# xandergos/terrain-diffusion

Hardware: AMD Instinct MI355X
Metric: terrain megapixels/sec (decoded) at fixed steps, 30m model (higher is better)
Workload: dtype bf16; 1 GPU; BASELINE configs[2]: terrain-diffusion-30m base U-Net, 8x8 tile grid (stride 32, 288x288 latents) with overlap blending, 20 steps, 64 windows batched per solver step; edm_steps=20, parallelism=1 independent streams (one process per GPU, no data-path collective)

## Files before the change

include/td_engine.h:

```cpp
#ifndef TD_ENGINE_H
#define TD_ENGINE_H
#include <stdint.h>

#ifdef __cplusplus
extern "C" {
#endif

typedef struct td_engine td_engine;
typedef struct td_unet td_unet;

enum { TD_OK = 0, TD_ERR_ARG = -1, TD_ERR_HIP = -2, TD_ERR_STATE = -3, TD_ERR_UNSUPPORTED = -4 };
enum { TD_DTYPE_F32 = 0, TD_DTYPE_BF16 = 1, TD_DTYPE_F16 = 2 };

typedef struct td_unet_config {
    int32_t image_size;
    int32_t in_channels, out_channels;
    int32_t model_channels;
    int32_t n_levels;
    int32_t channel_mults[8];
    int32_t layers_per_block[8];
    int32_t n_attn_resolutions;
    int32_t attn_resolutions[8];
    int32_t midblock_attention;
    float concat_balance;
    int32_t noise_emb_dims;
    int32_t emb_channels;
    int32_t n_cond;
    int32_t cond_type[8];
    int32_t cond_dims[8];
    float cond_weights[8];
} td_unet_config;

const char* td_last_error(void);
int td_version(void);
const char* td_build_id(void);

int td_engine_create(int device_id, td_engine** out);
void td_engine_destroy(td_engine* e);
int td_engine_synchronize(td_engine* e);
void* td_engine_stream(td_engine* e);
int td_engine_set_stream(td_engine* e, void* hip_stream);
int td_engine_set_option(td_engine* e, const char* key, int64_t value);

int td_engine_profile_read(td_engine* e, double* conv_ms, int64_t* conv_launches, double* other_ms, int64_t* other_launches, int reset);

int td_engine_profile_read_glds(td_engine* e, double* ms, double* flop, int64_t* launches, int reset);
int td_engine_profile_dump(td_engine* e, char* buf, int64_t capacity);

int td_unet_create(td_engine* e, const td_unet_config* cfg, int dtype, td_unet** out);
void td_unet_destroy(td_unet* u);
int td_unet_num_params(td_unet* u);
int td_unet_param_info(td_unet* u, int i, const char** name, int32_t* ndim, int64_t shape[4]);
int td_unet_set_param(td_unet* u, const char* name, const float* host_data, int64_t numel);
int td_unet_set_prefolded(td_unet* u, int prefolded);
int td_unet_finalize(td_unet* u);

int td_unet_cond_row_len(td_unet* u);
int td_unet_forward(td_unet* u, int n, int H, int W, const float* x, const float* t_host, const float* cond, float* out);

int td_unet_read_activation(td_unet* u, int n, int H, int W, const char* label, float* out_host, int64_t capacity, int32_t dims[4]);

uint64_t td_tile_seed(uint64_t base_seed, int64_t ty, int64_t tx);
int td_standard_normal(td_engine* e, uint64_t seed, int64_t n, float* out);
int td_noise_patches(td_engine* e, uint64_t base_seed, int n_windows, const int64_t* origins_host, int h, int w,
                     int channels, int tile_h, int tile_w, float scale, float* out);


int td_dpm_coefs(const float* sigmas_host, int n_steps, float sigma_data, int solver_order, int lower_order_final, float* out);

int td_sample_edm(td_unet* u, int n, int H, int W, int n_steps, const float* sigmas_host, float sigma_data,
                  const float* cond, float* x);
int td_sample_edm_guided(td_unet* u, td_unet* guide, float guidance_scale, int n, int H, int W, int n_steps, const float* sigmas_host,
                         float sigma_data, const float* cond, float* x);
int td_sample_consistency(td_unet* u, int n, int H, int W, float t, float sigma_data, const float* sample, const float* z,
                          const float* cond, float* out);
int td_sample_edm_img(td_unet* u, int n, int H, int W, int n_steps, const float* sigmas_host, float sigma_data, const float* cond,
                      const float* cond_img, int cimg_channels, float* x);
int td_sample_consistency_img(td_unet* u, int n, int H, int W, float t, float sigma_data, const float* sample, const float* z,
                              const float* cond, const float* cond_img, int cimg_channels, float* out);

int td_blend_windows(td_engine* e, float* canvas, int C, int Hc, int Wc, int size, int n_rows, const int32_t* row_starts_host,
                     int n_cols, const int32_t* col_starts_host, int n_tiles, const int32_t* wi_host, const int32_t* wj_host,
                     const float* tiles, int accumulate);

int td_gather_regions(td_engine* e, int C, int size, int n_regions, int h, int w, int maxk, const int32_t* desc_host, int n_windows,
                      const uint64_t* window_ptrs_host, float* out);
int td_blend_normalize(td_engine* e, const float* canvas, int C, int Hc, int Wc, float scale, float* out);
int td_linear_weight_window(td_engine* e, int size, float* out);

int td_resample2d(td_engine* e, const float* in, int C, int Hin, int Win, int Hout, int Wout, const int32_t* iy_host, const float* wy_host, int Ky,
                  const int32_t* ix_host, const float* wx_host, int Kx, float* out);
int td_residual_plus(td_engine* e, const float* packed, const float* lowres_up, int Hp, int Wp, float res_mean, float res_std, float* out);
int td_elev_finish(td_engine* e, const float* packed, const float* lowres_up, int Hp, int Wp, int oi, int oj, int h, int w, float res_mean,
                   float res_std, float* out);
int td_climate_finish(td_engine* e, const float* feats, int Hs, int Ws, const float* elev, int i1, int j1, int h, int w, float S, int ci1, int cj1, float* out);

int td_ddim_cfg_step(td_engine* e, const float* latent, const float* pred_uncond, const float* pred_cond, int64_t n, float guidance_scale, float alpha_t,
                     float alpha_prev, float* out);

int td_attention(td_engine* e, const float* q, const float* k, const float* v, int B, int H, int Lq, int Lk, int D, float scale, int normalize, float* out);

int td_perlin_map(td_engine* e, int rows, int cols, int i1, int j1, int seed, float frequency, int octaves, float lacunarity, float gain,
                  const float* src_quantiles, const float* dst_quantiles, int n_quantiles, float* out);

#ifdef __cplusplus
}
#endif
#endif
```

terrain_diffusion_amd/_lib.py:

```python
import ctypes as C
import os

_HERE = os.path.dirname(os.path.abspath(__file__))


class TdError(RuntimeError):
    pass


class Library:

    def __init__(self, file_name, sigs, last_error, label, missing="There is no CPU fallback."):
        self.path = os.path.join(_HERE, file_name)
        self.sigs, self.last_error, self.label, self.missing = sigs, last_error, label, missing
        self.handle = None

    def lib(self):
        if self.handle is None:
            if not os.path.exists(self.path):
                raise TdError(f"{self.path} is missing: build it first (python -c 'import __graft_entry__ as g; g.build()'). {self.missing}")
            l = C.CDLL(self.path)
            for name, (res, args) in self.sigs.items():
                fn = getattr(l, name)
                fn.restype = res
                fn.argtypes = args
            self.handle = l
        return self.handle

    def error_text(self):
        return getattr(self.lib(), self.last_error)().decode()

    def check(self, rc):
        if rc != 0:
            raise TdError(f"{self.label} error {rc}: {self.error_text()}")


class UnetConfig(C.Structure):
    _fields_ = [("image_size", C.c_int32), ("in_channels", C.c_int32), ("out_channels", C.c_int32),
                ("model_channels", C.c_int32), ("n_levels", C.c_int32), ("channel_mults", C.c_int32 * 8),
                ("layers_per_block", C.c_int32 * 8), ("n_attn_resolutions", C.c_int32),
                ("attn_resolutions", C.c_int32 * 8), ("midblock_attention", C.c_int32), ("concat_balance", C.c_float),
                ("noise_emb_dims", C.c_int32), ("emb_channels", C.c_int32), ("n_cond", C.c_int32),
                ("cond_type", C.c_int32 * 8), ("cond_dims", C.c_int32 * 8), ("cond_weights", C.c_float * 8)]


_P = C.c_void_p
_SIGS = {
    "td_last_error": (C.c_char_p, []),
    "td_version": (C.c_int, []),
    "td_build_id": (C.c_char_p, []),
    "td_engine_create": (C.c_int, [C.c_int, C.POINTER(_P)]),
    "td_engine_destroy": (None, [_P]),
    "td_engine_synchronize": (C.c_int, [_P]),
    "td_engine_stream": (_P, [_P]),
    "td_engine_set_stream": (C.c_int, [_P, _P]),
    "td_engine_set_option": (C.c_int, [_P, C.c_char_p, C.c_int64]),
    "td_engine_profile_read": (C.c_int, [_P, C.POINTER(C.c_double), C.POINTER(C.c_int64), C.POINTER(C.c_double), C.POINTER(C.c_int64), C.c_int]),
    "td_engine_profile_read_glds": (C.c_int, [_P, C.POINTER(C.c_double), C.POINTER(C.c_double), C.POINTER(C.c_int64), C.c_int]),
    "td_engine_profile_dump": (C.c_int, [_P, C.c_char_p, C.c_int64]),
    "td_unet_create": (C.c_int, [_P, C.POINTER(UnetConfig), C.c_int, C.POINTER(_P)]),
    "td_unet_destroy": (None, [_P]),
    "td_unet_num_params": (C.c_int, [_P]),
    "td_unet_param_info": (C.c_int, [_P, C.c_int, C.POINTER(C.c_char_p), C.POINTER(C.c_int32), C.POINTER(C.c_int64 * 4)]),
    "td_unet_set_param": (C.c_int, [_P, C.c_char_p, _P, C.c_int64]),
    "td_unet_set_prefolded": (C.c_int, [_P, C.c_int]),
    "td_unet_finalize": (C.c_int, [_P]),
    "td_unet_cond_row_len": (C.c_int, [_P]),
    "td_unet_forward": (C.c_int, [_P, C.c_int, C.c_int, C.c_int, _P, _P, _P, _P]),
    "td_unet_read_activation": (C.c_int, [_P, C.c_int, C.c_int, C.c_int, C.c_char_p, _P, C.c_int64, C.POINTER(C.c_int32 * 4)]),
    "td_dpm_coefs": (C.c_int, [_P, C.c_int, C.c_float, C.c_int, C.c_int, _P]),
    "td_tile_seed": (C.c_uint64, [C.c_uint64, C.c_int64, C.c_int64]),
    "td_standard_normal": (C.c_int, [_P, C.c_uint64, C.c_int64, _P]),
    "td_noise_patches": (C.c_int, [_P, C.c_uint64, C.c_int, _P, C.c_int, C.c_int, C.c_int, C.c_int, C.c_int, C.c_float, _P]),
    "td_sample_edm": (C.c_int, [_P, C.c_int, C.c_int, C.c_int, C.c_int, _P, C.c_float, _P, _P]),
    "td_sample_edm_guided": (C.c_int, [_P, _P, C.c_float, C.c_int, C.c_int, C.c_int, C.c_int, _P, C.c_float, _P, _P]),
    "td_sample_consistency": (C.c_int, [_P, C.c_int, C.c_int, C.c_int, C.c_float, C.c_float, _P, _P, _P, _P]),
    "td_sample_edm_img": (C.c_int, [_P, C.c_int, C.c_int, C.c_int, C.c_int, _P, C.c_float, _P, _P, C.c_int, _P]),
    "td_sample_consistency_img": (C.c_int, [_P, C.c_int, C.c_int, C.c_int, C.c_float, C.c_float, _P, _P, _P, _P, C.c_int, _P]),
    "td_blend_windows": (C.c_int, [_P, _P, C.c_int, C.c_int, C.c_int, C.c_int, C.c_int, _P, C.c_int, _P, C.c_int, _P, _P, _P, C.c_int]),
    "td_gather_regions": (C.c_int, [_P, C.c_int, C.c_int, C.c_int, C.c_int, C.c_int, C.c_int, _P, C.c_int, _P, _P]),
    "td_blend_normalize": (C.c_int, [_P, _P, C.c_int, C.c_int, C.c_int, C.c_float, _P]),
    "td_linear_weight_window": (C.c_int, [_P, C.c_int, _P]),
    "td_attention": (C.c_int, [_P, _P, _P, _P, C.c_int, C.c_int, C.c_int, C.c_int, C.c_int, C.c_float, C.c_int, _P]),
    "td_perlin_map": (C.c_int, [_P, C.c_int, C.c_int, C.c_int, C.c_int, C.c_int, C.c_float, C.c_int, C.c_float, C.c_float, _P, _P, C.c_int, _P]),
    "td_resample2d": (C.c_int, [_P, _P, C.c_int, C.c_int, C.c_int, C.c_int, C.c_int, _P, _P, C.c_int, _P, _P, C.c_int, _P]),
    "td_residual_plus": (C.c_int, [_P, _P, _P, C.c_int, C.c_int, C.c_float, C.c_float, _P]),
    "td_elev_finish": (C.c_int, [_P, _P, _P, C.c_int, C.c_int, C.c_int, C.c_int, C.c_int, C.c_int, C.c_float, C.c_float, _P]),
    "td_ddim_cfg_step": (C.c_int, [_P, _P, _P, _P, C.c_int64, C.c_float, C.c_float, C.c_float, _P]),
    "td_climate_finish": (C.c_int, [_P, _P, C.c_int, C.c_int, _P, C.c_int, C.c_int, C.c_int, C.c_int, C.c_float, C.c_int, C.c_int, _P]),
}
EXPORTS = tuple(_SIGS)

_LIB = Library("libtd_engine.so", _SIGS, "td_last_error", "td_engine")
LIB_PATH, lib, check = _LIB.path, _LIB.lib, _LIB.check
```

terrain_diffusion_amd/csrc/engine.hip:

```cpp
#include <hip/hip_runtime.h>
#include <math.h>
#include <stdio.h>
#include <string.h>

#include <map>
#include <memory>
#include <string>
#include <vector>
#include <unordered_map>

#include "../../include/td_engine.h"
#include "td_device.h"

#include "conv_igemm.hip"
#include "conv_glds.hip"
#include "conv_glds_wide.hip"
#include "conv_sb.hip"
#include "conv_s16.hip"
#include "conv_fewcout.hip"
#include "small_kernels.hip"
#include "compose_kernels.hip"
#include "attn_mfma.hip"

using namespace td;
// ... 824 lines not shown
    };

    const bool attn_on_mfma = u->dt == TD_DTYPE_BF16 && u->eng->option("attn_mfma", 1) != 0;
    auto attn_fits = [&](int tokens, const std::string& name) -> int {
        if (tokens > 64 && !attn_on_mfma)
            return fail(TD_ERR_UNSUPPORTED, "attention over more than 64 tokens needs bf16 mode with option attn_mfma = 1 (MFMA kernel; the scalar kernel holds 64): " + name);
        return TD_OK;
    };
    auto attn_workspace = [&](Op& a) -> int {
        if (!attn_on_mfma) return TD_OK;
        size_t qn, kn, vn;
        const size_t tot = attn_workspace_elems(N, a.C / 64, a.tokens, a.tokens, 64, &qn, &kn, &vn);
        void* ws;
        int r = new_buf(pl, tot * 2, &ws);
        if (r) return r;
        a.attn_ws = ws;
        return TD_OK;
    };

    Tensor xin;
    xin.C = chunk; xin.cstride = chunk; xin.H = H; xin.W = W;
    if ((rc = new_buf(pl, (size_t)N * H * W * chunk * es, &xin.ptr))) return rc;
    pl.xin = xin.ptr;

    std::vector<Tensor> skips;
    Tensor cur = xin;
    int h = H, w = W;
    for (size_t bi = 0; bi < u->enc.size(); ++bi) {
        const Block& b = u->enc[bi];
        bool next_norms = bi + 1 < u->enc.size() && u->enc[bi + 1].cin == u->enc[bi + 1].cout;
        Tensor o;
        if (b.is_conv) {
            if ((rc = conv(b.name, {{&cur, chunk, 9, 0, 0, 1.f}}, h, w, EPI_PLAIN, -1, nullptr, 0, false, 0.f, next_norms, false, &o))) return rc;
        } else {
            if (b.resample == 1) { h = (h + 1) / 2; w = (w + 1) / 2; }
            Tensor xs = cur;
            int rs = b.resample;
            if (b.cin != b.cout) {
                if ((rc = conv(b.name + ".conv_skip", {{&cur, b.cin, 1, rs, 0, 1.f}}, h, w, EPI_PLAIN, -1, nullptr, 0, false, 0.f, true, false, &xs))) return rc;
                rs = 0;
            }
            Tensor y1;
            if ((rc = conv(b.name + ".conv_res0", {{&xs, b.cout, 9, rs, 2, 1.f}}, h, w, EPI_EMB_SILU, b.cvec_off, nullptr, 0, false, 0.f, false, false, &y1))) return rc;
            if ((rc = conv(b.name + ".conv_res1", {{&y1, b.cout, 9, 0, 0, 1.f}}, h, w, EPI_RESIDUAL, -1, &xs, rs, true, b.attn ? 0.f : 256.f, next_norms && !b.attn, false, &o))) return rc;
            if (b.attn) {
                if ((rc = attn_fits(h * w, b.name))) return rc;
                Tensor qkv, att, o2;
                if ((rc = conv(b.name + ".attn_qkv", {{&o, b.cout, 1, 0, 0, 1.f}}, h, w, EPI_PLAIN, -1, nullptr, 0, false, 0.f, false, false, &qkv))) return rc;
                if ((rc = new_tensor(b.cout, h, w, false, 0, &att))) return rc;
                Op a; a.kind = Op::ATTN; a.qkv = qkv.ptr; a.att = att.ptr; a.tokens = h * w; a.C = b.cout; a.label = b.name + ".attn"; a.out_C = b.cout; a.out_H = h; a.out_W = w;
                if ((rc = attn_workspace(a))) return rc;
                pl.ops.push_back(a);
                if ((rc = conv(b.name + ".attn_proj", {{&att, b.cout, 1, 0, 0, 1.f}}, h, w, EPI_RESIDUAL, -1, &o, 0, false, 256.f, next_norms, false, &o2))) return rc;
                o = o2;
            }
        }
        cur = o;
        skips.push_back(o);
    }
    for (const Block& b : u->dec) {
        Tensor skip;
        if (b.concat) { skip = skips.back(); skips.pop_back(); }
        if (b.resample == 2) { h *= 2; w *= 2; }
        const int cx = b.cin - b.skip_c;
        float sa = 1.f, sb = 1.f;
        if (b.concat) {
            double t = u->cfg.concat_balance, wa = 1.0 - t, wb = t, C = sqrt((double)b.cin / (wa * wa + wb * wb));
            sa = (float)(C / sqrt((double)cx) * wa); sb = (float)(C / sqrt((double)b.skip_c) * wb);
        }
        std::vector<SegSpec> s0 = {{&cur, cx, 9, b.resample, 1, sa}};
        if (b.concat) s0.push_back({&skip, b.skip_c, 9, 0, 1, sb});
        Tensor y1, o;
        if ((rc = conv(b.name + ".conv_res0", s0, h, w, EPI_EMB_SILU, b.cvec_off, nullptr, 0, false, 0.f, false, false, &y1))) return rc;
        std::vector<SegSpec> s1 = {{&y1, b.cout, 9, 0, 0, 1.f}};
        const Tensor* res = nullptr;
        if (b.cin != b.cout) {
            s1.push_back({&cur, cx, 1, b.resample, 0, 1.f});
            if (b.concat) s1.push_back({&skip, b.skip_c, 1, 0, 0, 1.f});
        } else res = &cur;
        if ((rc = conv(b.name + ".conv_res1", s1, h, w, EPI_RESIDUAL, -1, res, b.resample, false, b.attn ? 0.f : 256.f, false, false, &o))) return rc;
        if (b.attn) {
            if ((rc = attn_fits(h * w, b.name))) return rc;
            Tensor qkv, att, o2;
            if ((rc = conv(b.name + ".attn_qkv", {{&o, b.cout, 1, 0, 0, 1.f}}, h, w, EPI_PLAIN, -1, nullptr, 0, false, 0.f, false, false, &qkv))) return rc;
            if ((rc = new_tensor(b.cout, h, w, false, 0, &att))) return rc;
            Op a; a.kind = Op::ATTN; a.qkv = qkv.ptr; a.att = att.ptr; a.tokens = h * w; a.C = b.cout; a.label = b.name + ".attn"; a.out_C = b.cout; a.out_H = h; a.out_W = w;
            if ((rc = attn_workspace(a))) return rc;
            pl.ops.push_back(a);
            if ((rc = conv(b.name + ".attn_proj", {{&att, b.cout, 1, 0, 0, 1.f}}, h, w, EPI_RESIDUAL, -1, &o, 0, false, 256.f, false, false, &o2))) return rc;
            o = o2;
        }
        cur = o;
    }
    Tensor Ft;
    if ((rc = conv("out_conv", {{&cur, u->final_c, 9, 0, 0, 1.f}}, h, w, EPI_PLAIN, -1, nullptr, 0, false, 0.f, false, true, &Ft))) return rc;
    pl.F = (float*)Ft.ptr;
    if (u->eng->option("producer_act", 1)) {
        std::unordered_map<const void*, size_t> producer;
        for (size_t k = 0; k < pl.ops.size(); ++k)
            if (pl.ops[k].kind == Op::CONV && !pl.ops[k].p.out_f32) producer[pl.ops[k].p.out] = k;
        for (size_t j = 0; j < pl.ops.size(); ++j) {
            if (pl.ops[j].kind != Op::CONV) continue;
            ConvParams& c = pl.ops[j].p;
            for (int i = 0; i < c.nseg; ++i) {
                if (c.seg[i].xform != 1) continue;
                auto it = producer.find(c.seg[i].src);
                if (it == producer.end() || it->second >= j) continue;
                ConvParams& q = pl.ops[it->second].p;
                if (q.out2 && q.out2_scale != c.seg[i].scale) continue;
                if (!q.out2) {
                    void* b2;
                    if ((rc = new_buf(pl, (size_t)q.N * q.H * q.W * q.out_cstride * es, &b2))) return rc;
                    q.out2 = b2; q.out2_scale = c.seg[i].scale;
                }
                c.seg[i].src = q.out2; c.seg[i].xform = 0; c.seg[i].scale = 1.f;
            }
        }
    }
    if (partial_bytes) {
        void* pp;
        if ((rc = new_buf(pl, partial_bytes, &pp))) return rc;
        pl.partial = (float*)pp;
        for (auto& op : pl.ops) if (op.kind == Op::CONV) op.p.partial = pl.partial;
    }
    const size_t xbytes = (size_t)N * std::max(u->cfg.in_channels, u->cfg.out_channels) * H * W * 4;
    pl.x.reset(new DevBuf()); pl.m1.reset(new DevBuf()); pl.m2.reset(new DevBuf()); pl.xt.reset(new DevBuf()); pl.cond.reset(new DevBuf());
    HIP_TRY(pl.x->alloc(xbytes)); HIP_TRY(pl.m1->alloc(xbytes)); HIP_TRY(pl.m2->alloc(xbytes)); HIP_TRY(pl.xt->alloc(xbytes));
    HIP_TRY(pl.cond->alloc((size_t)N * std::max(1, u->cond_row_len) * 4));
    HIP_TRY(hipDeviceSynchronize());
    pl.bytes += 4 * xbytes + (size_t)N * std::max(1, u->cond_row_len) * 4;
    pl.last_use = ++u->use_clock;
    *out = plp.get();
    u->plans[key] = std::move(plp);
    return TD_OK;
}

static int compute_cvecs(td_unet* u, Plan& pl, const std::vector<float>& t_steps, const float* d_cond) {
    hipStream_t st = u->eng->stream;
    const int rows = (int)t_steps.size() * pl.N;
    if (!pl.emb || pl.cvec_rows < rows) {
        pl.drop_graph();
        HIP_TRY(hipStreamSynchronize(st));
        pl.emb.reset(new DevBuf()); pl.cvec.reset(new DevBuf()); pl.tsteps.reset(new DevBuf());
        HIP_TRY(pl.emb->alloc((size_t)rows * u->emb_ch * 4));
        HIP_TRY(pl.cvec->alloc((size_t)rows * u->c_total * 4));
        HIP_TRY(pl.tsteps->alloc(std::max<size_t>(64, t_steps.size()) * 4));
        pl.cvec_rows = rows;
    }
    { int rc_ = upload(u->eng, pl.tsteps->p, t_steps.data(), t_steps.size() * 4); if (rc_) return rc_; }
    const int half = u->noise_dims / 2;
    hipLaunchKernelGGL(emb_kernel, dim3(rows, (u->emb_ch + 63) / 64), dim3(256), (size_t)(2 * half + u->embd.feat_total) * 4, st, (const float*)pl.tsteps->p, d_cond, pl.N,
                       (const float*)u->d_freqs->p, half, (const float*)u->d_wnoise->p, (const float*)u->d_wcond->p, (const float*)u->d_fourier->p,
                       u->embd, u->emb_ch, (float*)pl.emb->p);
    int max_cout = 64;
    for (auto& b : u->enc) max_cout = std::max(max_cout, b.cout);
    for (auto& b : u->dec) max_cout = std::max(max_cout, b.cout);
    bool c16 = u->emb_ch % 16 == 0 && u->c_total % 4 == 0;
    for (auto& b : u->enc) c16 = c16 && b.cout % 16 == 0;
    for (auto& b : u->dec) c16 = c16 && b.cout % 16 == 0;
    if (c16 && u->emb_ch % 64 == 0)
        hipLaunchKernelGGL(cvec_mfma_kernel<4>, dim3((max_cout + 63) / 64, (rows + 63) / 64, u->n_blocks), dim3(256), 0, st, (const float*)pl.emb->p, rows,
                           u->emb_ch, (const float*)u->d_wemb->p, (const int*)u->d_blk_woff->p, (const int*)u->d_blk_coff->p, (const int*)u->d_blk_cout->p,
                           u->c_total, (float*)pl.cvec->p);
    else if (c16)
        hipLaunchKernelGGL(cvec_mfma_kernel<1>, dim3((max_cout + 63) / 64, (rows + 63) / 64, u->n_blocks), dim3(256), 0, st, (const float*)pl.emb->p, rows,
                           u->emb_ch, (const float*)u->d_wemb->p, (const int*)u->d_blk_woff->p, (const int*)u->d_blk_coff->p, (const int*)u->d_blk_cout->p,
                           u->c_total, (float*)pl.cvec->p);
    else
    hipLaunchKernelGGL(cvec_kernel, dim3((max_cout + 63) / 64, (rows + 15) / 16, u->n_blocks), dim3(256), (size_t)16 * u->emb_ch * 4, st, (const float*)pl.emb->p, rows,
                       u->emb_ch, (const float*)u->d_wemb->p, (const int*)u->d_blk_woff->p, (const int*)u->d_blk_coff->p, (const int*)u->d_blk_cout->p,
                       u->c_total, (float*)pl.cvec->p);
    hipLaunchKernelGGL(cvec_norm_kernel, dim3(rows, u->n_blocks), dim3(256), 0, st, (float*)pl.cvec->p, (const int*)u->d_blk_coff->p,
                       (const int*)u->d_blk_cout->p, u->c_total);
    HIP_TRY(hipGetLastError());
    pl.cvec_written = rows;
    return TD_OK;
}

static int run_unet(td_unet* u, Plan& pl, int step, const SchedCoef* fuse = nullptr) {
    hipStream_t st = u->eng->stream;
    const float* cbase = (const float*)pl.cvec->p + (size_t)step * pl.N * u->c_total;
    const bool prof = u->eng->option("profile", 0) != 0;
    std::vector<hipEvent_t> evs;
    std::vector<int> ev_kind;
    std::vector<std::string> ev_label;
    std::vector<double> ev_flop;
    auto mark = [&]() { if (prof) { hipEvent_t e; (void)hipEventCreate(&e); (void)hipEventRecord(e, st); evs.push_back(e); } };
    struct Fin {
        td_unet* u; std::vector<hipEvent_t>& evs; std::vector<int>& kind; std::vector<std::string>& labels; std::vector<double>& flop; hipStream_t st;
        ~Fin() {
            if (evs.empty()) return;
            (void)hipStreamSynchronize(st);
            for (size_t i = 0; i + 1 < evs.size(); i += 2) {
                float ms = 0.f;
                (void)hipEventElapsedTime(&ms, evs[i], evs[i + 1]);
                auto& po = u->eng->prof_ops[labels[i / 2]]; po.first += ms; po.second++;
                if (flop[i / 2] > 0) { u->eng->prof_glds_ms += ms; u->eng->prof_glds_flop += flop[i / 2]; u->eng->prof_glds_launches++; }
                if (kind[i / 2] == 0) { u->eng->prof_conv_ms += ms; u->eng->prof_conv_launches++; } else { u->eng->prof_other_ms += ms; u->eng->prof_other_launches++; }
            }
            for (auto e : evs) (void)hipEventDestroy(e);
        }
    } fin{u, evs, ev_kind, ev_label, ev_flop, st};
    for (auto& op : pl.ops) {
        if (op.kind == Op::ATTN) {
            mark();
            if (op.attn_ws) {
                const int Hh = op.C / 64, L = op.tokens;
                size_t qn, kn, vn;
                attn_workspace_elems(pl.N, Hh, L, L, 64, &qn, &kn, &vn);
                __bf16 *Qp = (__bf16*)op.attn_ws, *Kp = Qp + qn, *Vt = Kp + kn;
                const __bf16* qkv = (const __bf16*)op.qkv;
                const AttnStrides so = {(long)L * op.C, 64L, (long)op.C, 1L};
                hipError_t ea = attn_pack_qkv64<__bf16>(qkv, 3L * op.C, pl.N, Hh, L, 0.125f, Qp, Kp, Vt, st);
                if (ea == hipSuccess) ea = attn_mfma(Qp, Kp, Vt, nullptr, (__bf16*)op.att, so, pl.N, Hh, L, L, 64, st);
                if (ea != hipSuccess) return fail(TD_ERR_HIP, std::string("attention launch: ") + hipGetErrorString(ea));
            } else
            TD_DISPATCH_T(u, hipLaunchKernelGGL(attn_kernel<T_>, dim3(pl.N, op.C / 64), dim3(256), 0, st, (const T_*)op.qkv, (T_*)op.att, op.tokens, op.C));
            mark(); if (prof) { ev_kind.push_back(1); ev_label.push_back(op.label); ev_flop.push_back(0.0); }
            HIP_TRY(hipGetLastError());
            continue;
        }
        ConvParams p = op.p;
        if (op.cvec_off >= 0) p.cvec = cbase + op.cvec_off;
        if (fuse && &op == &pl.ops.back()) {
            p.epi = EPI_DPM_STEP; p.dpm_x = (float*)pl.x->p; p.dpm_m1 = (float*)pl.m1->p; p.dpm_m2 = u->eng->option("solver_order", 2) == 3 ? (float*)pl.m2->p : nullptr; p.dpm_xin = pl.xin; p.dpm_xin_cstride = u->chunk; p.dpm_k = *fuse;
        }
        mark();
        hipError_t e = op.flavor == 6 ? launch_conv_fewcout(p, u->dt, st)
                       : op.flavor == 5 ? launch_conv_s16(p, u->dt, op.narrow, st)
                       : op.flavor == 4 ? launch_conv_sb(p, u->dt, op.narrow, op.sb_mt, op.sb_nt, st)
                       : op.flavor == 2 ? (op.glds_variant == 3 ? launch_conv_glds_wide(p, u->dt, op.bn, st) : launch_conv_glds(p, u->dt, op.narrow, op.bn, op.glds_variant, st))
                       : launch_conv(p, u->dt, op.narrow, op.bn, 0, st);
        mark(); if (prof) { ev_kind.push_back(0); char tag[160]; double gf_ = op.k_alg * 2.0 * p.N * p.H * p.W * p.Cout * 1e-9;
            double mb_ = 0.0; const double es_ = (double)u->esize();
            for (int si_ = 0; si_ < p.nseg; ++si_) mb_ += (double)p.N * p.seg[si_].Hs * p.seg[si_].Ws * p.seg[si_].C * es_ + (double)p.seg[si_].C / 64.0 * p.seg[si_].taps * p.CoutPad * 128.0 * (es_ / 2.0);
            if (p.res) mb_ += (double)p.N * p.res_Hs * p.res_Ws * p.Cout * es_;
            const double o1_ = (double)p.N * p.H * p.W * p.Cout * (p.out_f32 ? 4.0 : es_);
            const double mbs_ = (mb_ + o1_) * 1e-6;
            mb_ += o1_ * (p.out2 ? 2.0 : 1.0);
            mb_ *= 1e-6;
            snprintf(tag, sizeof tag, " [%dx%d k%d f%d%s bn%d wg%d ks%d gf%.2f mb%.2f mbs%.2f]", p.H, p.W, p.kgroups, op.flavor, op.flavor == 5 ? "c16" : op.flavor == 4 ? (op.sb_mt == 4 ? "m4n1" : op.sb_mt == 2 ? (op.sb_nt == 2 ? "m2n2" : "m2n1") : (op.sb_nt == 2 ? "m1n2" : "m1n1")) : op.flavor == 2 ? (op.glds_variant == 3 ? (p.persist > 0 ? "wp" : "w") : op.glds_variant == 2 ? "t" : op.glds_variant ? "s" : "b") : "", op.bn, p.n_ntiles * p.tiles_x * p.tiles_y * p.img_groups, p.ksplit, gf_, mb_, mbs_); ev_label.push_back(op.label + tag);
            ev_flop.push_back(op.flavor == 2 ? 2.0 * p.N * p.H * p.W * (double)p.Cout * op.k_alg : 0.0); }
        if (e != hipSuccess) return fail(TD_ERR_HIP, "conv launch " + op.label + ": " + hipGetErrorString(e));
    }
    return TD_OK;
}

static inline dim3 grid1(size_t n, int b = 256) { return dim3((unsigned)((n + b - 1) / b)); }

extern "C" {

const char* td_last_error(void) { return g_err.c_str(); }
int td_version(void) { return 1; }
#ifndef TD_CSRC_SHA
#define TD_CSRC_SHA "unstamped"
#endif
const char* td_build_id(void) { return TD_CSRC_SHA; }

int td_engine_create(int device_id, td_engine** out) {
    if (!out) return fail(TD_ERR_ARG, "null out");
    int ndev = 0;
    if (hipGetDeviceCount(&ndev) != hipSuccess || ndev == 0) return fail(TD_ERR_HIP, "no HIP device visible: the engine has no CPU fallback");
    if (device_id < 0 || device_id >= ndev) return fail(TD_ERR_ARG, "bad device id");
    DevGuard dg_(device_id);
    td_engine* e = new td_engine();
    e->device = device_id;
    { hipDeviceProp_t prop; if (hipGetDeviceProperties(&prop, device_id) == hipSuccess && prop.multiProcessorCount > 0) e->n_cus = prop.multiProcessorCount; }
    hipError_t err = hipStreamCreateWithFlags(&e->stream, hipStreamNonBlocking);
    e->own_stream = e->stream;
    if (err == hipSuccess) err = hipStreamCreateWithFlags(&e->stream2, hipStreamNonBlocking);
    if (err == hipSuccess) err = hipEventCreateWithFlags(&e->ev_fork, hipEventDisableTiming);
    if (err == hipSuccess) err = hipEventCreateWithFlags(&e->ev_join, hipEventDisableTiming);
    if (err == hipSuccess) err = hipMalloc(&e->zeros, 4096);
    if (err == hipSuccess) err = hipMemset(e->zeros, 0, 4096);
    if (err == hipSuccess) err = hipDeviceSynchronize();
    if (err != hipSuccess) { if (e->stream) (void)hipStreamDestroy(e->stream); if (e->stream2) (void)hipStreamDestroy(e->stream2); if (e->ev_fork) (void)hipEventDestroy(e->ev_fork); if (e->ev_join) (void)hipEventDestroy(e->ev_join); delete e; return fail(TD_ERR_HIP, hipGetErrorString(err)); }
    *out = e;
    return TD_OK;
}
void td_engine_destroy(td_engine* e) {
    if (!e) return;
    DevGuard dg_(e->device);
    if (e->own_stream) { (void)hipStreamSynchronize(e->stream); (void)hipStreamDestroy(e->own_stream); }
    if (e->stream2) (void)hipStreamDestroy(e->stream2);
    if (e->ev_fork) (void)hipEventDestroy(e->ev_fork);
    if (e->ev_join) (void)hipEventDestroy(e->ev_join);
    if (e->zeros) (void)hipFree(e->zeros);
    delete e;
}
int td_engine_synchronize(td_engine* e) {
    DevGuard dg_(e->device); HIP_TRY(hipStreamSynchronize(e->stream)); e->deferred.clear(); e->ring.reset(); return TD_OK; }
void* td_engine_stream(td_engine* e) { return (void*)e->stream; }
int td_engine_set_stream(td_engine* e, void* hip_stream) {
    if (!e) return fail(TD_ERR_ARG, "null engine");
    DevGuard dg_(e->device);
    HIP_TRY(hipStreamSynchronize(e->stream));
    e->deferred.clear();
    e->ring.reset();
    e->stream = hip_stream ? (hipStream_t)hip_stream : e->own_stream;
    return TD_OK;
}
static const char* const kKnownOptions[] = {
    "async", "batch_invariant", "fuse_solver", "graph", "lower_order_final", "profile", "solver_order", "dual_stream", "dual_stream_min_batch", "sampler_stop_after",
    "plan_cache_mb", "plan_cache_max",
    "attn_mfma", "bn128_min_wgs", "glds", "glds_bn", "glds_bn64", "glds_dma1x1", "glds_min_wgs", "glds_round_aware", "glds_small_max_groups",
    "glds_splitk", "glds_splitk_from_groups", "glds_splitk_max", "glds_splitk_min_groups", "glds_tiny", "glds_variant", "glds_wide", "glds_wide_min_wgs", "glds_wide_tail", "glds_wide_persist", "fewcout",
    "producer_act", "s16", "s16_min_wgs", "sb", "sb_m4", "sb_max_glds_wgs", "sb_mt", "sb_nt", "sb_order", "sb_splitk", "sb_splitk_max", "sb_splitk_wgs", "sb_target_wgs", "splitk",
    "splitk_target_wgs", "splitk_weighted", "walk_alternate"};
int td_engine_set_option(td_engine* e, const char* key, int64_t value) {
    if (!e || !key) return fail(TD_ERR_ARG, "null");
    bool known = false;
    for (const char* k : kKnownOptions) known = known || strcmp(k, key) == 0;
    if (!known) return fail(TD_ERR_ARG, std::string("unknown engine option \"") + key + "\" (include/td_engine.h lists the options)");
    e->opt[key] = value;
    return TD_OK;
}

int td_engine_profile_read(td_engine* e, double* conv_ms, int64_t* conv_launches, double* other_ms, int64_t* other_launches, int reset) {
    if (conv_ms) *conv_ms = e->prof_conv_ms;
    if (conv_launches) *conv_launches = e->prof_conv_launches;
    if (other_ms) *other_ms = e->prof_other_ms;
    if (other_launches) *other_launches = e->prof_other_launches;
    if (reset) { e->prof_conv_ms = e->prof_other_ms = 0.0; e->prof_conv_launches = e->prof_other_launches = 0; e->prof_ops.clear(); }
    return TD_OK;
}
int td_engine_profile_read_glds(td_engine* e, double* ms, double* flop, int64_t* launches, int reset) {
    if (ms) *ms = e->prof_glds_ms;
    if (flop) *flop = e->prof_glds_flop;
    if (launches) *launches = e->prof_glds_launches;
    if (reset) { e->prof_glds_ms = e->prof_glds_flop = 0.0; e->prof_glds_launches = 0; }
    return TD_OK;
}
int td_engine_profile_dump(td_engine* e, char* buf, int64_t capacity) {
    std::string out;
    for (auto& kv : e->prof_ops) {
        char line[256];
        snprintf(line, sizeof line, "%s\t%.4f\t%lld\n", kv.first.c_str(), kv.second.first, (long long)kv.second.second);
        out += line;
    }
    if ((int64_t)out.size() + 1 > capacity) return fail(TD_ERR_ARG, "capacity");
    memcpy(buf, out.c_str(), out.size() + 1);
    return TD_OK;
}

int td_unet_create(td_engine* e, const td_unet_config* cfg, int dtype, td_unet** out) {
    if (!e || !cfg || !out) return fail(TD_ERR_ARG, "null argument");
    if (dtype != TD_DTYPE_F32 && dtype != TD_DTYPE_BF16 && dtype != TD_DTYPE_F16) return fail(TD_ERR_ARG, "dtype");
    std::unique_ptr<td_unet> u(new td_unet());
    u->eng = e; u->cfg = *cfg; u->dt = dtype; u->bf16 = dtype != TD_DTYPE_F32; u->chunk = u->bf16 ? 64 : 32;
    int rc = build_blocks(u.get());
    if (rc) return rc;
    *out = u.release();
    return TD_OK;
}
void td_unet_destroy(td_unet* u) {
    if (!u) return;
    DevGuard dg_(u->eng->device);
    (void)hipStreamSynchronize(u->eng->stream);
    delete u;
}
int td_unet_num_params(td_unet* u) { return (int)u->params.size(); }
int td_unet_param_info(td_unet* u, int i, const char** name, int32_t* ndim, int64_t shape[4]) {
    if (i < 0 || i >= (int)u->params.size()) return fail(TD_ERR_ARG, "index");
    *name = u->params[i].name.c_str(); *ndim = u->params[i].ndim;
    for (int k = 0; k < 4; ++k) shape[k] = u->params[i].shape[k];
    return TD_OK;
}
int td_unet_set_param(td_unet* u, const char* name, const float* host_data, int64_t numel) {
    if (u->finalized) return fail(TD_ERR_STATE, "already finalized");
    auto it = u->pindex.find(name);
    if (it == u->pindex.end()) return fail(TD_ERR_ARG, std::string("unknown parameter ") + name);
    Param& p = u->params[it->second];
    if (numel != p.numel()) return fail(TD_ERR_ARG, std::string("size mismatch for ") + name);
    p.data.assign(host_data, host_data + numel);
    p.set = true;
    return TD_OK;
}
int td_unet_set_prefolded(td_unet* u, int prefolded) {
    if (u->finalized) return fail(TD_ERR_STATE, "already finalized");
    u->prefolded = prefolded != 0;
    return TD_OK;
}
int td_unet_finalize(td_unet* u) {
    DevGuard dg_(u->eng->device);
    if (u->finalized) return TD_OK;
    return finalize(u);
}

int td_unet_cond_row_len(td_unet* u) { return u->cond_row_len; }

int td_unet_forward(td_unet* u, int n, int H, int W, const float* x, const float* t_host, const float* cond, float* out) {
    DevGuard dg_(u->eng->device);
    if (!u->finalized) return fail(TD_ERR_STATE, "finalize first");
    Plan* pl;
    int rc = build_plan(u, n, H, W, &pl);
    if (rc) return rc;
    td_engine* e = u->eng;
    hipStream_t st = e->stream;
    const int C = u->cfg.in_channels, Co = u->cfg.out_channels, HW = H * W;
    std::vector<Buf> hold;
    const void *dx, *dcond = nullptr;
    if ((rc = to_device(e, x, (size_t)n * C * HW * 4, hold, &dx))) return rc;
    if (u->cond_row_len > 0 && (rc = to_device(e, cond, (size_t)n * u->cond_row_len * 4, hold, &dcond))) return rc;
    OutStage os;
    if ((rc = out_device(e, out, (size_t)n * Co * HW * 4, hold, &os))) return rc;
    std::vector<float> ts(t_host, t_host + n);
    bool uniform = true;
    for (int i = 1; i < n; ++i) uniform = uniform && ts[i] == ts[0];
    if (uniform) {
        if ((rc = compute_cvecs(u, *pl, std::vector<float>(1, ts[0]), (const float*)dcond))) return rc;
    } else {
        if ((rc = compute_cvecs(u, *pl, ts, (const float*)dcond))) return rc;
        for (int i = 1; i < n; ++i) {
            HIP_TRY(hipMemcpyAsync((float*)pl->cvec->p + (size_t)i * u->c_total, (float*)pl->cvec->p + ((size_t)i * n + i) * u->c_total, (size_t)u->c_total * 4,
                                   hipMemcpyDeviceToDevice, st));
            HIP_TRY(hipMemcpyAsync((float*)pl->emb->p + (size_t)i * u->emb_ch, (float*)pl->emb->p + ((size_t)i * n + i) * u->emb_ch, (size_t)u->emb_ch * 4,
                                   hipMemcpyDeviceToDevice, st));
        }
    }
    TD_DISPATCH_T(u, hipLaunchKernelGGL(prep_input_kernel<T_>, grid1((size_t)n * HW), dim3(256), 0, st, (const float*)dx, (T_*)pl->xin, n, C, HW, u->chunk, 1.f, C));
    if ((rc = run_unet(u, *pl, 0))) return rc;
    hipLaunchKernelGGL(unpack_output_kernel, grid1((size_t)n * HW), dim3(256), 0, st, (const float*)pl->F, (float*)os.dev, n, Co, HW, 8, 1.f);
    HIP_TRY(hipGetLastError());
    if ((rc = out_finish(e, os))) return rc;
    HIP_TRY(hipStreamSynchronize(st));
    return TD_OK;
}

int td_unet_read_activation(td_unet* u, int n, int H, int W, const char* label, float* out_host, int64_t capacity, int32_t dims[4]) {
    DevGuard dg_(u->eng->device);
    Plan* pl;
    int rc = build_plan(u, n, H, W, &pl);
    if (rc) return rc;
    if (!strcmp(label, "@emb") || !strcmp(label, "@cvec")) {
        const bool is_emb = !strcmp(label, "@emb");
        const int width = is_emb ? u->emb_ch : u->c_total;
        dims[0] = n; dims[1] = width; dims[2] = 1; dims[3] = 1;
        if ((int64_t)n * width > capacity) return fail(TD_ERR_ARG, "capacity");
        HIP_TRY(hipStreamSynchronize(u->eng->stream));
        HIP_TRY(hipMemcpy(out_host, is_emb ? pl->emb->p : pl->cvec->p, (size_t)n * width * 4, hipMemcpyDeviceToHost));
        return TD_OK;
    }
    if (!strcmp(label, "@emb:rows") || !strcmp(label, "@cvec:rows")) {
        const bool is_emb = !strcmp(label, "@emb:rows");
        const int width = is_emb ? u->emb_ch : u->c_total, rows = pl->cvec_written;
        if (rows < 1 || !pl->emb) return fail(TD_ERR_STATE, "no embedding rows on this plan yet: run a forward or a sampler call first");
        dims[0] = rows; dims[1] = width; dims[2] = 1; dims[3] = 1;
        if ((int64_t)rows * width > capacity) return fail(TD_ERR_ARG, "capacity");
        HIP_TRY(hipStreamSynchronize(u->eng->stream));
        HIP_TRY(hipMemcpy(out_host, is_emb ? pl->emb->p : pl->cvec->p, (size_t)rows * width * 4, hipMemcpyDeviceToHost));
        return TD_OK;
    }
    if (!strcmp(label, "@x") || !strcmp(label, "@m1") || !strcmp(label, "@m2") || !strcmp(label, "@xt")) {
        const int C = u->cfg.out_channels;
        const Buf& b = !strcmp(label, "@x") ? pl->x : !strcmp(label, "@m1") ? pl->m1 : !strcmp(label, "@m2") ? pl->m2 : pl->xt;
        dims[0] = n; dims[1] = C; dims[2] = H; dims[3] = W;
        if ((int64_t)n * C * H * W > capacity) return fail(TD_ERR_ARG, "capacity");
        HIP_TRY(hipStreamSynchronize(u->eng->stream));
        HIP_TRY(hipMemcpy(out_host, b->p, (size_t)n * C * H * W * 4, hipMemcpyDeviceToHost));
        return TD_OK;
    }
    if (!strcmp(label, "@xin")) {
        const int cs = u->chunk;
        const size_t HW = (size_t)H * W, elems = (size_t)n * HW * cs;
        dims[0] = n; dims[1] = cs; dims[2] = H; dims[3] = W;
        if ((int64_t)elems > capacity) return fail(TD_ERR_ARG, "capacity");
        HIP_TRY(hipStreamSynchronize(u->eng->stream));
        std::vector<uint8_t> raw(elems * (u->bf16 ? 2 : 4));
        HIP_TRY(hipMemcpy(raw.data(), pl->xin, raw.size(), hipMemcpyDeviceToHost));
        for (int i = 0; i < n; ++i)
            for (int c = 0; c < cs; ++c)
                for (size_t p = 0; p < HW; ++p) {
                    const size_t src = ((size_t)i * HW + p) * cs + c;
                    float v;
                    if (!u->bf16) v = ((const float*)raw.data())[src];
                    else if (u->dt == TD_DTYPE_F16) { _Float16 h; memcpy(&h, (const uint16_t*)raw.data() + src, 2); v = (float)h; }
                    else { uint32_t b = (uint32_t)((const uint16_t*)raw.data())[src] << 16; memcpy(&v, &b, 4); }
                    out_host[((size_t)i * cs + c) * HW + p] = v;
                }
        return TD_OK;
    }
    if (!strncmp(label, "sumsq:", 6)) {
        for (auto& op : pl->ops) {
            if (op.kind != Op::CONV || op.label != label + 6 || !op.p.out_sumsq) continue;
            const int parts = op.p.ksplit > 1 ? (op.p.CoutPad + 255) / 256 : (op.flavor >= 2 ? op.p.CoutPad / 32 : op.p.n_ntiles * 2);
            const size_t M = (size_t)n * op.out_H * op.out_W;
            dims[0] = parts; dims[1] = n; dims[2] = op.out_H; dims[3] = op.out_W;
            if ((int64_t)(parts * M) > capacity) return fail(TD_ERR_ARG, "capacity");
            HIP_TRY(hipStreamSynchronize(u->eng->stream));
            HIP_TRY(hipMemcpy(out_host, op.p.out_sumsq, parts * M * 4, hipMemcpyDeviceToHost));
            return TD_OK;
        }
        return fail(TD_ERR_ARG, "no sumsq for that op");
    }
    for (auto& op : pl->ops) {
        if (op.label != label) continue;
        const bool is_attn = op.kind == Op::ATTN;
        const int C = op.out_C, h = op.out_H, w = op.out_W, cs = is_attn ? op.C : op.p.out_cstride;
        dims[0] = n; dims[1] = C; dims[2] = h; dims[3] = w;
        if ((int64_t)n * C * h * w > capacity) return fail(TD_ERR_ARG, "capacity");
        HIP_TRY(hipStreamSynchronize(u->eng->stream));
        const size_t elems = (size_t)n * h * w * cs;
        const bool f32out = (!is_attn && op.p.out_f32) || !u->bf16;
        std::vector<uint8_t> raw(elems * (f32out ? 4 : 2));
        HIP_TRY(hipMemcpy(raw.data(), is_attn ? op.att : op.p.out, raw.size(), hipMemcpyDeviceToHost));
        for (int i = 0; i < n; ++i)
            for (int c = 0; c < C; ++c)
                for (int p = 0; p < h * w; ++p) {
                    size_t src = ((size_t)i * h * w + p) * cs + c;
                    float v;
                    if (f32out) v = ((const float*)raw.data())[src];
                    else if (u->dt == TD_DTYPE_F16) { _Float16 h; memcpy(&h, (const uint16_t*)raw.data() + src, 2); v = (float)h; }
                    else { uint32_t b = (uint32_t)((const uint16_t*)raw.data())[src] << 16; memcpy(&v, &b, 4); }
                    out_host[((size_t)i * C + c) * h * w + p] = v;
                }
        return TD_OK;
    }
    return fail(TD_ERR_ARG, std::string("no conv or attention op labelled ") + label);
}

static void dpm_coefs(const float* sig, int n_steps, float sigma_data, int solver_order, bool lower_order_final, std::vector<SchedCoef>& ks) {
    ks.resize(n_steps);
    int lower = 0;
    for (int i = 0; i < n_steps; ++i) {
        SchedCoef k;
        const float s = sig[i], st = sig[i + 1], sd = sigma_data;
        k.c_skip = (sd * sd) / (s * s + sd * sd);
        k.c_out = s * sd / sqrtf(s * s + sd * sd);
        const bool final = (i == n_steps - 1);
        const bool second = (i == n_steps - 2) && lower_order_final && n_steps < 15;
        k.order = (solver_order < 2 || lower < 1 || final) ? 1 : ((solver_order == 2 || lower < 2 || second) ? 2 : 3);
        const float lam_t = 0.f - logf(st), lam_s = 0.f - logf(s);
        const float h = lam_t - lam_s;
        k.a = st / s;
        k.b0 = expf(-h) - 1.0f;
        k.inv_r0 = 0.f; k.inv_r1 = 0.f; k.f01 = 0.f; k.inv_r01 = 0.f; k.c1 = 0.f; k.c2 = 0.f;
        if (k.order >= 2) {
            const float lam_s1 = 0.f - logf(sig[i - 1]);
            const float h0 = lam_s - lam_s1;
            const float r0 = h0 / h;
            k.inv_r0 = 1.0f / r0;
            if (k.order == 3) {
                const float lam_s2 = 0.f - logf(sig[i - 2]);
                const float r1 = (lam_s1 - lam_s2) / h;
                k.inv_r1 = 1.0f / r1; k.f01 = r0 / (r0 + r1); k.inv_r01 = 1.0f / (r0 + r1);
                k.c1 = (expf(-h) - 1.0f) / h + 1.0f;
                k.c2 = (expf(-h) - 1.0f + h) / (h * h) - 0.5f;
            }
        }
        k.last = final ? 1 : 0;
        k.c_in_next = final ? 0.f : 1.f / sqrtf(st * st + sd * sd);
        if (lower < solver_order) ++lower;
        ks[i] = k;
    }
}

int td_dpm_coefs(const float* sigmas_host, int n_steps, float sigma_data, int solver_order, int lower_order_final, float* out) {
    if (!sigmas_host || !out || n_steps < 1) return fail(TD_ERR_ARG, "td_dpm_coefs: null argument or n_steps < 1");
    if (solver_order < 1 || solver_order > 3) return fail(TD_ERR_ARG, "solver_order must be 1, 2 or 3");
    std::vector<SchedCoef> ks;
    dpm_coefs(sigmas_host, n_steps, sigma_data, solver_order, lower_order_final != 0, ks);
    for (int i = 0; i < n_steps; ++i) {
        const SchedCoef& k = ks[i];
        const float row[13] = {k.c_skip, k.c_out, k.a, k.b0, k.inv_r0, k.inv_r1, k.f01, k.inv_r01, k.c1, k.c2, k.c_in_next, (float)k.order, (float)k.last};
        memcpy(out + (size_t)i * 13, row, sizeof row);
    }
    return TD_OK;
}

static int stage_cond_img(td_unet* u, Plan& pl, int n, int HW, const float* cond_img, int cimg, int Cs, std::vector<Buf>& hold) {
    if (cimg == 0) return TD_OK;
    if (!cond_img) return fail(TD_ERR_ARG, "cond_img is null");
    const void* dimg;
    int rc = to_device(u->eng, cond_img, (size_t)n * cimg * HW * 4, hold, &dimg);
    if (rc) return rc;
    hipStream_t st = u->eng->stream;
    TD_DISPATCH_T(u, hipLaunchKernelGGL(write_cond_img_kernel<T_>, grid1((size_t)n * HW), dim3(256), 0, st, (const float*)dimg, (T_*)pl.xin, n, cimg, HW, u->chunk, Cs));
    HIP_TRY(hipGetLastError());
    return TD_OK;
}

static int sample_edm_lane(td_unet* u, td_unet* guide, float gscale, int n, int H, int W, int n_steps, const float* sigmas_host, float sigma_data,
                           const float* cond, const float* cond_img, int cimg, float* x, int lane, std::vector<Buf>& hold) {
    if (guide) {
        if (!guide->finalized) return fail(TD_ERR_STATE, "finalize the guide model first");
        if (guide->eng != u->eng || guide->dt != u->dt) return fail(TD_ERR_ARG, "guide model must live on the same engine and use the same dtype");
        if (guide->cfg.in_channels != u->cfg.in_channels || guide->cfg.out_channels != u->cfg.out_channels || guide->cond_row_len != u->cond_row_len)
            return fail(TD_ERR_ARG, "guide model must take the same inputs as the main model");
    }
    if (!u->finalized) return fail(TD_ERR_STATE, "finalize first");
    if (n_steps < 1) return fail(TD_ERR_ARG, "n_steps");
    Plan* pl;
    int rc = build_plan(u, n, H, W, &pl, lane);
    if (rc) return rc;
    td_engine* e = u->eng;
    hipStream_t st = e->stream;
    const int Cin = u->cfg.in_channels, C = u->cfg.out_channels, HW = H * W;
    if (C + cimg != Cin) return fail(TD_ERR_ARG, "in_channels must equal out_channels + conditioning-image channels");
    const size_t xbytes = (size_t)n * C * HW * 4;
    const bool x_dev = is_device_ptr(x);
    HIP_TRY(hipMemcpyAsync(pl->x->p, x, xbytes, x_dev ? hipMemcpyDeviceToDevice : hipMemcpyHostToDevice, st));
    if (u->cond_row_len > 0) {
        const size_t cb = (size_t)n * u->cond_row_len * 4;
        HIP_TRY(hipMemcpyAsync(pl->cond->p, cond, cb, is_device_ptr(cond) ? hipMemcpyDeviceToDevice : hipMemcpyHostToDevice, st));
    }
    if ((rc = stage_cond_img(u, *pl, n, HW, cond_img, cimg, C, hold))) return rc;
    std::vector<float> ts(n_steps);
    for (int i = 0; i < n_steps; ++i) ts[i] = atanf(sigmas_host[i] / sigma_data);
    if ((rc = compute_cvecs(u, *pl, ts, (const float*)pl->cond->p))) return rc;
    Plan* gpl = nullptr;
    if (guide) {
        if ((rc = build_plan(guide, n, H, W, &gpl, lane))) return rc;
        if ((rc = stage_cond_img(guide, *gpl, n, HW, cond_img, cimg, C, hold))) return rc;
        if ((rc = compute_cvecs(guide, *gpl, ts, (const float*)pl->cond->p))) return rc;
    }
    std::vector<SchedCoef> ks;
    const int solver_order = (int)e->option("solver_order", 2);
    if (solver_order < 1 || solver_order > 3) return fail(TD_ERR_ARG, "solver_order must be 1, 2 or 3");
    const bool lof = e->option("lower_order_final", 1) != 0;
    dpm_coefs(sigmas_host, n_steps, sigma_data, solver_order, lof, ks);
    const float c_in0 = 1.f / sqrtf(sigmas_host[0] * sigmas_host[0] + sigma_data * sigma_data);
    const int stop_after = (int)e->option("sampler_stop_after", -1);
    const int n_run = stop_after >= 0 ? std::min(stop_after, n_steps) : n_steps;
    if (stop_after >= 0) {
        HIP_TRY(hipMemsetAsync(pl->m1->p, 0, xbytes, st));
        HIP_TRY(hipMemsetAsync(pl->m2->p, 0, xbytes, st));
    }

    auto enqueue = [&]() -> int {
        TD_DISPATCH_T(u, hipLaunchKernelGGL(prep_input_kernel<T_>, grid1((size_t)n * HW), dim3(256), 0, st, (const float*)pl->x->p, (T_*)pl->xin, n, C, HW, u->chunk, c_in0, Cin));
        if (gpl) {
            TD_DISPATCH_T(u, hipLaunchKernelGGL(prep_input_kernel<T_>, grid1((size_t)n * HW), dim3(256), 0, st, (const float*)pl->x->p, (T_*)gpl->xin, n, C, HW, u->chunk, c_in0, Cin));
        }
        const float* Fg = gpl ? (const float*)gpl->F : nullptr;
        const bool fuse = !gpl && e->option("fuse_solver", 1) != 0 && pl->ops.back().kind == Op::CONV && pl->ops.back().p.epi == EPI_PLAIN && pl->ops.back().p.out_f32;
        for (int i = 0; i < n_run; ++i) {
            int r = run_unet(u, *pl, i, fuse ? &ks[i] : nullptr);
            if (r) return r;
            if (fuse) continue;
            if (gpl && (r = run_unet(guide, *gpl, i))) return r;
            TD_DISPATCH_T(u, hipLaunchKernelGGL(dpm_step_kernel<T_>, grid1((size_t)n * HW), dim3(256), 0, st, (float*)pl->x->p, (float*)pl->m1->p, (const float*)pl->F, (T_*)pl->xin, n, C, HW, 8, u->chunk, ks[i], Fg, gscale, gpl ? (T_*)gpl->xin : (T_*)nullptr, solver_order == 3 ? (float*)pl->m2->p : (float*)nullptr));
        }
        HIP_TRY(hipGetLastError());
        return TD_OK;
    };

    const bool use_graph = e->option("graph", 1) != 0 && e->option("profile", 0) == 0;
    if (use_graph) {
        std::vector<float> sg(sigmas_host, sigmas_host + n_steps + 1);
        const void* gkey = gpl ? (const void*)gpl->cvec->p : nullptr;
        if (!pl->graph || pl->graph_sigmas != sg || pl->graph_sigma_data != sigma_data || pl->graph_solver_order != solver_order || pl->graph_lof != (int)lof ||
            pl->graph_guide != (const void*)gpl || pl->graph_guide_cvec != gkey || pl->graph_gscale != gscale || pl->graph_fuse != (int)e->option("fuse_solver", 1) ||
            pl->graph_stop != stop_after) {
            pl->drop_graph();
            hipGraph_t g = nullptr;
            HIP_TRY(hipStreamBeginCapture(st, hipStreamCaptureModeThreadLocal));
            rc = enqueue();
            hipError_t ce = hipStreamEndCapture(st, &g);
            if (rc) { if (g) (void)hipGraphDestroy(g); return rc; }
            if (ce != hipSuccess) return fail(TD_ERR_HIP, std::string("graph capture: ") + hipGetErrorString(ce));
            hipError_t ie = hipGraphInstantiate(&pl->graph, g, nullptr, nullptr, 0);
            (void)hipGraphDestroy(g);
            if (ie != hipSuccess) { pl->graph = nullptr; return fail(TD_ERR_HIP, std::string("graph instantiate: ") + hipGetErrorString(ie)); }
            pl->graph_sigmas = sg; pl->graph_sigma_data = sigma_data; pl->graph_solver_order = solver_order; pl->graph_lof = (int)lof; pl->graph_fuse = (int)e->option("fuse_solver", 1);
            pl->graph_stop = stop_after;
            pl->graph_guide = gpl; pl->graph_guide_cvec = gkey; pl->graph_gscale = gscale;
        }
        HIP_TRY(hipGraphLaunch(pl->graph, st));
    } else if ((rc = enqueue())) return rc;
    HIP_TRY(hipMemcpyAsync(x, pl->x->p, xbytes, x_dev ? hipMemcpyDeviceToDevice : hipMemcpyDeviceToHost, st));
    return TD_OK;
}

static int sample_edm_impl(td_unet* u, td_unet* guide, float gscale, int n, int H, int W, int n_steps, const float* sigmas_host, float sigma_data,
                           const float* cond, const float* cond_img, int cimg, float* x) {
    td_engine* e = u->eng;
    DevGuard dg_(e->device);
    std::vector<Buf> hold;
    const bool dual = e->stream2 && e->option("dual_stream", 1) != 0 && n >= std::max<int64_t>(2, e->option("dual_stream_min_batch", 32));
    const bool concurrent = e->option("profile", 0) == 0;
    const bool all_dev = is_device_ptr(x) && (!cond || is_device_ptr(cond)) && (!cond_img || is_device_ptr(cond_img));
    if (!dual) {
        int rc = sample_edm_lane(u, guide, gscale, n, H, W, n_steps, sigmas_host, sigma_data, cond, cond_img, cimg, x, 0, hold);
        if (rc) { (void)hipStreamSynchronize(e->stream); return rc; }
        return end_call(e, hold, all_dev);
    }
    const int nA = n / 2, nB = n - nA, C = u->cfg.out_channels;
    const size_t HW = (size_t)H * W;
    if (concurrent) { HIP_TRY(hipEventRecord(e->ev_fork, e->stream)); HIP_TRY(hipStreamWaitEvent(e->stream2, e->ev_fork, 0)); }
    int rc = sample_edm_lane(u, guide, gscale, nA, H, W, n_steps, sigmas_host, sigma_data, cond, cond_img, cimg, x, 0, hold);
    if (!rc) {
        if (concurrent) std::swap(e->stream, e->stream2);
        rc = sample_edm_lane(u, guide, gscale, nB, H, W, n_steps, sigmas_host, sigma_data, cond ? cond + (size_t)nA * u->cond_row_len : nullptr,
                             cond_img ? cond_img + (size_t)nA * cimg * HW : nullptr, cimg, x + (size_t)nA * C * HW, 1, hold);
        if (concurrent) std::swap(e->stream, e->stream2);
    }
    if (rc) { (void)hipStreamSynchronize(e->stream); (void)hipStreamSynchronize(e->stream2); return rc; }
    if (concurrent) { HIP_TRY(hipEventRecord(e->ev_join, e->stream2)); HIP_TRY(hipStreamWaitEvent(e->stream, e->ev_join, 0)); }
    return end_call(e, hold, all_dev);
}

int td_sample_edm_img(td_unet* u, int n, int H, int W, int n_steps, const float* sigmas_host, float sigma_data, const float* cond,
                      const float* cond_img, int cimg, float* x) {
    return sample_edm_impl(u, nullptr, 1.f, n, H, W, n_steps, sigmas_host, sigma_data, cond, cond_img, cimg, x);
}
int td_sample_edm(td_unet* u, int n, int H, int W, int n_steps, const float* sigmas_host, float sigma_data, const float* cond, float* x) {
    return sample_edm_impl(u, nullptr, 1.f, n, H, W, n_steps, sigmas_host, sigma_data, cond, nullptr, 0, x);
}
int td_sample_edm_guided(td_unet* u, td_unet* guide, float guidance_scale, int n, int H, int W, int n_steps, const float* sigmas_host, float sigma_data,
                         const float* cond, float* x) {
    if (!guide) return fail(TD_ERR_ARG, "null guide model");
    return sample_edm_impl(u, guide, guidance_scale, n, H, W, n_steps, sigmas_host, sigma_data, cond, nullptr, 0, x);
}

int td_sample_consistency_img(td_unet* u, int n, int H, int W, float t, float sigma_data, const float* sample, const float* z, const float* cond,
                              const float* cond_img, int cimg, float* out) {
    DevGuard dg_(u->eng->device);
    if (!u->finalized) return fail(TD_ERR_STATE, "finalize first");
    Plan* pl;
    int rc = build_plan(u, n, H, W, &pl);
    if (rc) return rc;
    td_engine* e = u->eng;
    hipStream_t st = e->stream;
    const int Cin = u->cfg.in_channels, C = u->cfg.out_channels, HW = H * W;
    if (C + cimg != Cin) return fail(TD_ERR_ARG, "in_channels must equal out_channels + conditioning-image channels");
    const size_t xbytes = (size_t)n * C * HW * 4;
    std::vector<Buf> hold;
    const void* dz;
    if ((rc = to_device(e, z, xbytes, hold, &dz))) return rc;
    if (sample) HIP_TRY(hipMemcpyAsync(pl->x->p, sample, xbytes, is_device_ptr(sample) ? hipMemcpyDeviceToDevice : hipMemcpyHostToDevice, st));
    else HIP_TRY(hipMemsetAsync(pl->x->p, 0, xbytes, st));
    if (u->cond_row_len > 0)
        HIP_TRY(hipMemcpyAsync(pl->cond->p, cond, (size_t)n * u->cond_row_len * 4, is_device_ptr(cond) ? hipMemcpyDeviceToDevice : hipMemcpyHostToDevice, st));
    if ((rc = stage_cond_img(u, *pl, n, HW, cond_img, cimg, C, hold))) return rc;
    if ((rc = compute_cvecs(u, *pl, std::vector<float>(1, t), (const float*)pl->cond->p))) return rc;
    OutStage os;
    if ((rc = out_device(e, out, xbytes, hold, &os))) return rc;
    const float ct = cosf(t), sn = sinf(t);
    TD_DISPATCH_T(u, hipLaunchKernelGGL(consistency_pre_kernel<T_>, grid1((size_t)n * HW), dim3(256), 0, st, (const float*)pl->x->p, (const float*)dz, (float*)pl->xt->p, (T_*)pl->xin, n, C, HW, u->chunk, ct, sn, sigma_data, Cin));
    if ((rc = run_unet(u, *pl, 0))) return rc;
    hipLaunchKernelGGL(consistency_post_kernel, grid1((size_t)n * HW), dim3(256), 0, st, (const float*)pl->xt->p, (const float*)pl->F, (float*)os.dev, n, C, HW, 8, ct, sn, sigma_data);
    HIP_TRY(hipGetLastError());
    if ((rc = out_finish(e, os))) return rc;
    return end_call(e, hold, !os.host && is_device_ptr(z) && (!sample || is_device_ptr(sample)) && (!cond || is_device_ptr(cond)) && (!cond_img || is_device_ptr(cond_img)));
}

int td_sample_consistency(td_unet* u, int n, int H, int W, float t, float sigma_data, const float* sample, const float* z, const float* cond, float* out) {
    return td_sample_consistency_img(u, n, H, W, t, sigma_data, sample, z, cond, nullptr, 0, out);
}

uint64_t td_tile_seed(uint64_t base_seed, int64_t ty, int64_t tx) {
    const uint64_t G = 0x9E3779B9ULL;
    uint64_t h = base_seed * G;
    h = h + ((uint64_t)ty & 0xFFFFFFFFULL);
    h = h * G + ((uint64_t)tx & 0xFFFFFFFFULL);
    return h;
}

int td_standard_normal(td_engine* e, uint64_t seed, int64_t n, float* out) {
    DevGuard dg_(e->device);
    if (n <= 0) return TD_OK;
    std::vector<Buf> hold;
    OutStage os;
    int rc;
    if ((rc = out_device(e, out, (size_t)n * 4, hold, &os))) return rc;
    Buf sd(new DevBuf());
    HIP_TRY(sd->alloc(8, false));
    HIP_TRY(hipMemcpyAsync(sd->p, &seed, 8, hipMemcpyHostToDevice, e->stream));
    hipLaunchKernelGGL(noise_tiles_kernel, dim3(1), dim3(256), 0, e->stream, (const uint64_t*)sd->p, (float*)os.dev, n);
    HIP_TRY(hipGetLastError());
    if ((rc = out_finish(e, os))) return rc;
    HIP_TRY(hipStreamSynchronize(e->stream));
    return TD_OK;
}

static inline int64_t fdiv(int64_t a, int64_t b) { int64_t q = a / b; return (a % b != 0 && ((a < 0) != (b < 0))) ? q - 1 : q; }

int td_noise_patches(td_engine* e, uint64_t base_seed, int n_windows, const int64_t* origins, int h, int w, int channels, int tile_h, int tile_w,
                     float scale, float* out) {
    DevGuard dg_(e->device);
    if (n_windows <= 0) return TD_OK;
    if (h > tile_h || w > tile_w) return fail(TD_ERR_UNSUPPORTED, "window larger than the noise tile");
    std::map<std::pair<int64_t, int64_t>, int> slot;
    std::vector<uint64_t> seeds;
    std::vector<int> index((size_t)n_windows * 4, 0), org((size_t)n_windows * 2);
    for (int i = 0; i < n_windows; ++i) {
        const int64_t y0 = origins[2 * i], x0 = origins[2 * i + 1];
        org[2 * i] = (int)y0; org[2 * i + 1] = (int)x0;
        const int64_t ty0 = fdiv(y0, tile_h), ty1 = fdiv(y0 + h - 1, tile_h), tx0 = fdiv(x0, tile_w), tx1 = fdiv(x0 + w - 1, tile_w);
        for (int64_t ty = ty0; ty <= ty1; ++ty)
            for (int64_t tx = tx0; tx <= tx1; ++tx) {
                auto key = std::make_pair(ty, tx);
                auto it = slot.find(key);
                int s;
                if (it == slot.end()) { s = (int)seeds.size(); slot[key] = s; seeds.push_back(td_tile_seed(base_seed, ty, tx)); } else s = it->second;
                index[(size_t)i * 4 + (ty - ty0) * 2 + (tx - tx0)] = s;
            }
    }
    const int64_t tn = (int64_t)channels * tile_h * tile_w;
    Buf dseeds(new DevBuf()), dtiles(new DevBuf()), dindex(new DevBuf()), dorg(new DevBuf());
    HIP_TRY(dseeds->scratch(e->scratch, seeds.size() * 8)); HIP_TRY(dtiles->scratch(e->scratch, seeds.size() * tn * 4));
    HIP_TRY(dindex->scratch(e->scratch, index.size() * 4)); HIP_TRY(dorg->scratch(e->scratch, org.size() * 4));
    hipStream_t st = e->stream;
    int rc;
    if ((rc = upload(e, dseeds->p, seeds.data(), seeds.size() * 8)) || (rc = upload(e, dindex->p, index.data(), index.size() * 4)) ||
        (rc = upload(e, dorg->p, org.data(), org.size() * 4))) return rc;
    std::vector<Buf> hold;
    OutStage os;
    if ((rc = out_device(e, out, (size_t)n_windows * channels * h * w * 4, hold, &os))) return rc;
    hipLaunchKernelGGL(noise_tiles_kernel, dim3((unsigned)seeds.size()), dim3(256), 0, st, (const uint64_t*)dseeds->p, (float*)dtiles->p, tn);
    hipLaunchKernelGGL(noise_gather_kernel, dim3((channels * h * w + 255) / 256, n_windows), dim3(256), 0, st, (const float*)dtiles->p, (const int*)dindex->p,
                       (const int*)dorg->p, (float*)os.dev, channels, h, w, tile_h, tile_w, scale);
    HIP_TRY(hipGetLastError());
    if ((rc = out_finish(e, os))) return rc;
    return end_call(e, hold, !os.host);
}

static void weight_window_host(int size, std::vector<float>& w) {
    w.resize((size_t)size * size);
    const float mid = (float)((size - 1) / 2.0);
    const float k = (float)(1 - 1e-3);
    std::vector<float> a(size);
    for (int i = 0; i < size; ++i) {
        float d = fabsf((float)i - mid) / mid;
        d = fminf(fmaxf(d, 0.f), 1.f);
        a[i] = 1.f - k * d;
    }
    for (int y = 0; y < size; ++y)
        for (int x = 0; x < size; ++x) w[(size_t)y * size + x] = a[y] * a[x];
}

int td_linear_weight_window(td_engine* e, int size, float* out) {
    DevGuard dg_(e->device);
    std::vector<float> w;
    weight_window_host(size, w);
    HIP_TRY(hipMemcpy(out, w.data(), w.size() * 4, is_device_ptr(out) ? hipMemcpyHostToDevice : hipMemcpyHostToHost));
    return TD_OK;
}

int td_blend_windows(td_engine* e, float* canvas, int C, int Hc, int Wc, int size, int n_rows, const int32_t* row_starts, int n_cols,
                     const int32_t* col_starts, int n_tiles, const int32_t* wi, const int32_t* wj, const float* tiles, int accumulate) {
    DevGuard dg_(e->device);
    if (C + 1 > 8) return fail(TD_ERR_UNSUPPORTED, "C+1 must be <= 8");
    hipStream_t st = e->stream;
    std::vector<int> rowmap((size_t)Hc * 4, -1), colmap((size_t)Wc * 4, -1), tile_of((size_t)n_rows * n_cols, -1);
    for (int ic = 0; ic < n_rows; ++ic)
        for (int y = std::max(0, row_starts[ic]); y < std::min(Hc, row_starts[ic] + size); ++y) {
            int k = 0;
            while (k < 4 && rowmap[(size_t)y * 4 + k] >= 0) ++k;
            if (k == 4) return fail(TD_ERR_UNSUPPORTED, "more than 4 windows cover a canvas row");
            rowmap[(size_t)y * 4 + k] = ic;
        }
    for (int jc = 0; jc < n_cols; ++jc)
        for (int x = std::max(0, col_starts[jc]); x < std::min(Wc, col_starts[jc] + size); ++x) {
            int k = 0;
            while (k < 4 && colmap[(size_t)x * 4 + k] >= 0) ++k;
            if (k == 4) return fail(TD_ERR_UNSUPPORTED, "more than 4 windows cover a canvas column");
            colmap[(size_t)x * 4 + k] = jc;
        }
    for (int i = 0; i < n_tiles; ++i) {
        if (wi[i] < 0 || wi[i] >= n_rows || wj[i] < 0 || wj[i] >= n_cols) return fail(TD_ERR_ARG, "window index out of range");
        tile_of[(size_t)wi[i] * n_cols + wj[i]] = i;
    }
    std::vector<float> ww;
    weight_window_host(size, ww);
    auto up = [&](const void* src, size_t bytes, Buf& b) -> int {
        b.reset(new DevBuf());
        HIP_TRY(b->scratch(e->scratch, bytes));
        return upload(e, b->p, src, bytes);
    };
    Buf drow, dcol, drs, dcs, dtof, dww;
    int rc;
    if ((rc = up(rowmap.data(), rowmap.size() * 4, drow)) || (rc = up(colmap.data(), colmap.size() * 4, dcol)) || (rc = up(row_starts, (size_t)n_rows * 4, drs)) ||
        (rc = up(col_starts, (size_t)n_cols * 4, dcs)) || (rc = up(tile_of.data(), tile_of.size() * 4, dtof)) || (rc = up(ww.data(), ww.size() * 4, dww)))
        return rc;
    std::vector<Buf> hold;
    const void* dt;
    if ((rc = to_device(e, tiles, (size_t)n_tiles * C * size * size * 4, hold, &dt))) return rc;
    const size_t cbytes = (size_t)(C + 1) * Hc * Wc * 4;
    float* dcanvas = canvas;
    Buf cstage;
    const bool cdev = is_device_ptr(canvas);
    if (!cdev) {
        cstage.reset(new DevBuf());
        HIP_TRY(cstage->scratch(e->scratch, cbytes));
        dcanvas = (float*)cstage->p;
        if (accumulate) HIP_TRY(hipMemcpyAsync(dcanvas, canvas, cbytes, hipMemcpyHostToDevice, st));
    }
    hipLaunchKernelGGL(blend_gather_kernel, grid1((size_t)Hc * Wc), dim3(256), 0, st, (const float*)dt, (const float*)dww->p, dcanvas, C, Hc, Wc, size,
                       (const int*)drow->p, (const int*)dcol->p, (const int*)drs->p, (const int*)dcs->p, (const int*)dtof->p, n_cols, accumulate);
    HIP_TRY(hipGetLastError());
    if (!cdev) HIP_TRY(hipMemcpyAsync(canvas, dcanvas, cbytes, hipMemcpyDeviceToHost, st));
    return end_call(e, hold, cdev && is_device_ptr(tiles));
}

int td_gather_regions(td_engine* e, int C, int size, int n_regions, int h, int w, int maxk, const int32_t* desc_host, int n_windows,
                      const uint64_t* window_ptrs_host, float* out) {
    DevGuard dg_(e->device);
    if (C + 1 > 8) return fail(TD_ERR_UNSUPPORTED, "C+1 must be <= 8");
    if (n_regions <= 0) return TD_OK;
    if (maxk < 1 || h < 1 || w < 1 || n_windows < 0 || !is_device_ptr(out)) return fail(TD_ERR_ARG, "td_gather_regions: bad shape / host output");
    for (size_t i = 0; i < (size_t)n_regions * maxk; ++i)
        if (desc_host[i * 3] >= n_windows) return fail(TD_ERR_ARG, "td_gather_regions: window slot out of range");
    hipStream_t st = e->stream;
    auto& ww = e->wwin[size];
    if (!ww) {
        std::vector<float> hw;
        weight_window_host(size, hw);
        ww.reset(new DevBuf());
        HIP_TRY(ww->alloc(hw.size() * 4, false));
        HIP_TRY(hipMemcpy(ww->p, hw.data(), hw.size() * 4, hipMemcpyHostToDevice));
    }
    const size_t dbytes = (size_t)n_regions * maxk * 3 * 4, pbytes = ((size_t)n_windows * 8 + 15) / 16 * 16;
    Buf stage(new DevBuf());
    HIP_TRY(stage->scratch(e->scratch, pbytes + dbytes));
    unsigned char* stg = (unsigned char*)stage->p;
    int rc;
    if ((rc = upload(e, stg, window_ptrs_host, (size_t)n_windows * 8)) || (rc = upload(e, stg + pbytes, desc_host, dbytes))) return rc;
    hipLaunchKernelGGL(regions_gather_kernel, dim3((unsigned)(((size_t)h * w + 255) / 256), (unsigned)n_regions), dim3(256), 0, st, (const float* const*)stg,
                       (const int*)(stg + pbytes), maxk, (const float*)ww->p, out, C, h, w, size);
    HIP_TRY(hipGetLastError());
    std::vector<Buf> hold;
    hold.push_back(std::move(stage));
    return end_call(e, hold, true);
}

int td_blend_normalize(td_engine* e, const float* canvas, int C, int Hc, int Wc, float scale, float* out) {
    DevGuard dg_(e->device);
    std::vector<Buf> hold;
    const void* dc;
    int rc;
    if ((rc = to_device(e, canvas, (size_t)(C + 1) * Hc * Wc * 4, hold, &dc))) return rc;
    OutStage os;
    if ((rc = out_device(e, out, (size_t)C * Hc * Wc * 4, hold, &os))) return rc;
    hipLaunchKernelGGL(blend_normalize_kernel, grid1((size_t)Hc * Wc), dim3(256), 0, e->stream, (const float*)dc, (float*)os.dev, C, Hc * Wc, scale);
    HIP_TRY(hipGetLastError());
    if ((rc = out_finish(e, os))) return rc;
    return end_call(e, hold, !os.host && is_device_ptr(canvas));
}

int td_resample2d(td_engine* e, const float* in, int C, int Hin, int Win, int Hout, int Wout, const int32_t* iy, const float* wy, int Ky,
                  const int32_t* ix, const float* wx, int Kx, float* out) {
    DevGuard dg_(e->device);
    if (C < 1 || Hin < 1 || Win < 1 || Hout < 1 || Wout < 1 || Ky < 1 || Kx < 1) return fail(TD_ERR_ARG, "td_resample2d: bad geometry");
    for (int i = 0; i < Hout * Ky; ++i) if (iy[i] < 0 || iy[i] >= Hin) return fail(TD_ERR_ARG, "td_resample2d: row tap out of range");
    for (int i = 0; i < Wout * Kx; ++i) if (ix[i] < 0 || ix[i] >= Win) return fail(TD_ERR_ARG, "td_resample2d: column tap out of range");
    hipStream_t st = e->stream;
    std::vector<Buf> hold;
    const void *din, *diy, *dwy, *dix, *dwx;
    int rc;
    if ((rc = to_device(e, in, (size_t)C * Hin * Win * 4, hold, &din)) || (rc = to_device(e, iy, (size_t)Hout * Ky * 4, hold, &diy)) ||
        (rc = to_device(e, wy, (size_t)Hout * Ky * 4, hold, &dwy)) || (rc = to_device(e, ix, (size_t)Wout * Kx * 4, hold, &dix)) ||
        (rc = to_device(e, wx, (size_t)Wout * Kx * 4, hold, &dwx))) return rc;
    OutStage os;
    if ((rc = out_device(e, out, (size_t)C * Hout * Wout * 4, hold, &os))) return rc;
    Buf tmp(new DevBuf());
    HIP_TRY(tmp->scratch(e->scratch, (size_t)C * Hin * Wout * 4));
    hipLaunchKernelGGL(resample_rows_kernel, grid1((size_t)C * Hin * Wout), dim3(256), 0, st, (const float*)din, (float*)tmp->p, C, Hin, Win, Wout, (const int*)dix, (const float*)dwx, Kx);
    hipLaunchKernelGGL(resample_cols_kernel, grid1((size_t)C * Hout * Wout), dim3(256), 0, st, (const float*)tmp->p, (float*)os.dev, C, Hin, Hout, Wout, (const int*)diy, (const float*)dwy, Ky);
    HIP_TRY(hipGetLastError());
    if ((rc = out_finish(e, os))) return rc;
    hold.push_back(std::move(tmp));
    return end_call(e, hold, !os.host && is_device_ptr(in));
}

int td_residual_plus(td_engine* e, const float* packed, const float* lowres_up, int Hp, int Wp, float res_mean, float res_std, float* out) {
    DevGuard dg_(e->device);
    if (!is_device_ptr(packed) || !is_device_ptr(lowres_up) || !is_device_ptr(out)) return fail(TD_ERR_ARG, "td_residual_plus: device buffers only");
    hipLaunchKernelGGL(residual_plus_kernel, grid1((size_t)Hp * Wp), dim3(256), 0, e->stream, packed, lowres_up, out, Hp * Wp, res_mean, res_std);
    HIP_TRY(hipGetLastError());
    std::vector<Buf> none;
    return end_call(e, none, true);
}

int td_elev_finish(td_engine* e, const float* packed, const float* lowres_up, int Hp, int Wp, int oi, int oj, int h, int w, float res_mean, float res_std, float* out) {
    DevGuard dg_(e->device);
    if (!is_device_ptr(packed) || !is_device_ptr(lowres_up) || !is_device_ptr(out)) return fail(TD_ERR_ARG, "td_elev_finish: device buffers only");
    if (oi < 0 || oj < 0 || oi + h > Hp || oj + w > Wp) return fail(TD_ERR_ARG, "td_elev_finish: crop outside the window");
    hipLaunchKernelGGL(elev_finish_kernel, grid1((size_t)h * w), dim3(256), 0, e->stream, packed, lowres_up, out, Hp, Wp, oi, oj, h, w, res_mean, res_std);
    HIP_TRY(hipGetLastError());
    std::vector<Buf> none;
    return end_call(e, none, true);
}

int td_ddim_cfg_step(td_engine* e, const float* latent, const float* pred_uncond, const float* pred_cond, int64_t n, float guidance_scale, float alpha_t,
                     float alpha_prev, float* out) {
    DevGuard dg_(e->device);
    if (n < 1 || !(alpha_t > 0.f) || !(alpha_t <= 1.f) || !(alpha_prev > 0.f) || !(alpha_prev <= 1.f)) return fail(TD_ERR_ARG, "td_ddim_cfg_step: bad arguments");
    if (!is_device_ptr(latent) || !is_device_ptr(pred_uncond) || !is_device_ptr(pred_cond) || !is_device_ptr(out)) return fail(TD_ERR_ARG, "td_ddim_cfg_step: device buffers only");
    hipLaunchKernelGGL(ddim_cfg_step_kernel, grid1((size_t)n), dim3(256), 0, e->stream, latent, pred_uncond, pred_cond, out, (size_t)n, guidance_scale,
                       sqrtf(1.f - alpha_t), sqrtf(alpha_t), sqrtf(alpha_prev), sqrtf(1.f - alpha_prev));
    HIP_TRY(hipGetLastError());
    std::vector<Buf> none;
    return end_call(e, none, true);
}

int td_climate_finish(td_engine* e, const float* feats, int Hs, int Ws, const float* elev, int i1, int j1, int h, int w, float S, int ci1, int cj1, float* out) {
    DevGuard dg_(e->device);
    if (!is_device_ptr(feats) || !is_device_ptr(elev) || !is_device_ptr(out)) return fail(TD_ERR_ARG, "td_climate_finish: device buffers only");
    if (Hs < 1 || Ws < 1 || h < 1 || w < 1 || !(S > 0.f)) return fail(TD_ERR_ARG, "td_climate_finish: bad geometry");
    hipLaunchKernelGGL(climate_finish_kernel, grid1((size_t)h * w), dim3(256), 0, e->stream, feats, elev, out, Hs, Ws, i1, j1, h, w, S, ci1, cj1);
    HIP_TRY(hipGetLastError());
    std::vector<Buf> none;
    return end_call(e, none, true);
}

int td_perlin_map(td_engine* e, int rows, int cols, int i1, int j1, int seed, float frequency, int octaves, float lacunarity, float gain,
                  const float* src_quantiles, const float* dst_quantiles, int n_quantiles, float* out) {
    DevGuard dg_(e->device);
    if (rows < 1 || cols < 1 || octaves < 1 || octaves > 16 || n_quantiles < 2) return fail(TD_ERR_ARG, "td_perlin_map: bad arguments");
    std::vector<Buf> hold;
    const void *ds, *dd;
    int rc;
    if ((rc = to_device(e, src_quantiles, (size_t)n_quantiles * 4, hold, &ds)) || (rc = to_device(e, dst_quantiles, (size_t)n_quantiles * 4, hold, &dd))) return rc;
    OutStage os;
    if ((rc = out_device(e, out, (size_t)rows * cols * 4, hold, &os))) return rc;
    hipLaunchKernelGGL(perlin_map_kernel, grid1((size_t)rows * cols), dim3(256), 0, e->stream, (float*)os.dev, rows, cols, i1, j1, seed, frequency, octaves, lacunarity, gain,
                       (const float*)ds, (const float*)dd, n_quantiles);
    HIP_TRY(hipGetLastError());
    if ((rc = out_finish(e, os))) return rc;
    HIP_TRY(hipStreamSynchronize(e->stream));
    return TD_OK;
}

int td_attention(td_engine* e, const float* q, const float* k, const float* v, int B, int H, int Lq, int Lk, int D, float scale, int normalize, float* out) {
    DevGuard dg_(e->device);
    if (B < 1 || H < 1 || Lq < 1 || Lk < 1 || D < 1 || D > 160) return fail(TD_ERR_ARG, "td_attention: 1 <= D <= 160, positive sizes");
    hipStream_t st = e->stream;
    std::vector<Buf> hold;
    const void *dq, *dk, *dv;
    int rc;
    if ((rc = to_device(e, q, (size_t)B * H * Lq * D * 4, hold, &dq)) || (rc = to_device(e, k, (size_t)B * H * Lk * D * 4, hold, &dk)) ||
        (rc = to_device(e, v, (size_t)B * H * Lk * D * 4, hold, &dv))) return rc;
    OutStage os;
    if ((rc = out_device(e, out, (size_t)B * H * Lq * D * 4, hold, &os))) return rc;
    size_t qn, kn, vn;
    const size_t tot = attn_workspace_elems(B, H, Lq, Lk, D, &qn, &kn, &vn);
    Buf ws(new DevBuf());
    HIP_TRY(ws->alloc(tot * 2, false));
    __bf16 *Qp = (__bf16*)ws->p, *Kp = Qp + qn, *Vt = Kp + kn;
    const AttnStrides sq = {(long)H * Lq * D, (long)Lq * D, (long)D, 1L}, sk = {(long)H * Lk * D, (long)Lk * D, (long)D, 1L};
    HIP_TRY(attn_pack<float>((const float*)dq, (const float*)dk, (const float*)dv, sq, sk, sk, B, H, Lq, Lk, D, normalize, scale, Qp, Kp, Vt, st));
    HIP_TRY(attn_mfma(Qp, Kp, Vt, (float*)os.dev, nullptr, sq, B, H, Lq, Lk, D, st));
    if ((rc = out_finish(e, os))) return rc;
    HIP_TRY(hipStreamSynchronize(st));
    return TD_OK;
}

}
```

terrain_diffusion_amd/csrc/small_kernels.hip:

```cpp
#include "td_device.h"

namespace td {

typedef __bf16 bf16x8 __attribute__((ext_vector_type(8)));
typedef __bf16 bf16x4 __attribute__((ext_vector_type(4)));
typedef float f32x4 __attribute__((ext_vector_type(4)));

__device__ __forceinline__ float mp_silu_acc(float x) { return x / (1.f + expf(-x)) * (1.f / 0.596f); }

__device__ __forceinline__ float wave_sum(float v) {
#pragma unroll
    for (int o = 32; o >= 1; o >>= 1) v += __shfl_xor(v, o);
    return v;
}

struct EmbDesc {
    int n, row_len, feat_total;
    int type[8], dims[8], xoff[8], foff[8], woff[8], froff[8];
    float weight[8];
    float inv_norm;
};
__global__ __launch_bounds__(256) void emb_kernel(const float* __restrict__ t_steps, const float* __restrict__ cond, int n_tiles,
                                                  const float* __restrict__ freqs, int half, const float* __restrict__ w_noise,
                                                  const float* __restrict__ w_cond, const float* __restrict__ fourier, EmbDesc d, int emb_ch,
// ... 117 lines not shown
        if (r < rows) *(f32x4*)(craw + (size_t)r * c_total + blk_coff[blk] + co0 + 4 * lg) = acc[nb] + 1.f;
    }
}

__global__ __launch_bounds__(256) void cvec_norm_kernel(float* __restrict__ c, const int* __restrict__ blk_coff, const int* __restrict__ blk_cout, int c_total) {
    __shared__ float red[4];
    const int blk = blockIdx.y, cout = blk_cout[blk];
    float* v = c + (size_t)blockIdx.x * c_total + blk_coff[blk];
    float s = 0.f;
    for (int i = threadIdx.x; i < cout; i += blockDim.x) s += v[i] * v[i];
    s = wave_sum(s);
    if ((threadIdx.x & 63) == 0) red[threadIdx.x >> 6] = s;
    __syncthreads();
    const float tot = red[0] + red[1] + red[2] + red[3];
    const float inv = 1.f / sqrtf(tot / (float)cout + 1e-8f);
    for (int i = threadIdx.x; i < cout; i += blockDim.x) v[i] *= inv;
}

template <typename T>
__global__ __launch_bounds__(256) void attn_kernel(const T* __restrict__ qkv, T* __restrict__ out, int tokens, int C) {
    __shared__ float sq[64][65], sk[64][65], sv[64][65], sw[64][65];
    const int n = blockIdx.x, head = blockIdx.y, tid = threadIdx.x;
    const size_t base = (size_t)n * tokens * 3 * C;
    for (int e = tid; e < tokens * 64; e += 256) {
        int tok = e >> 6, c = e & 63;
        const T* ptr = qkv + base + (size_t)tok * 3 * C + (head * 64 + c) * 3;
        sq[tok][c] = (float)ptr[0]; sk[tok][c] = (float)ptr[1]; sv[tok][c] = (float)ptr[2];
    }
    __syncthreads();
    if (tid < 3 * 64) {
        int which = tid >> 6, tok = tid & 63;
        if (tok < tokens) {
            float (*m)[65] = which == 0 ? sq : (which == 1 ? sk : sv);
            float s = 0.f;
            for (int c = 0; c < 64; ++c) s += m[tok][c] * m[tok][c];
            float inv = 1.f / (1e-4f + sqrtf(s) * 0.125f);
            if (which == 1) inv *= 0.125f;
            for (int c = 0; c < 64; ++c) m[tok][c] *= inv;
        }
    }
    __syncthreads();
    const int q = tid >> 2, part = tid & 3;
    float mx = -3.0e38f;
    if (q < tokens) {
        for (int k = part; k < tokens; k += 4) {
            float s = 0.f;
            for (int c = 0; c < 64; ++c) s += sq[q][c] * sk[k][c];
            sw[q][k] = s;
            mx = fmaxf(mx, s);
        }
    }
    mx = fmaxf(mx, __shfl_xor(mx, 1)); mx = fmaxf(mx, __shfl_xor(mx, 2));
    float den = 0.f;
    if (q < tokens) {
        for (int k = part; k < tokens; k += 4) { float e = expf(sw[q][k] - mx); sw[q][k] = e; den += e; }
    }
    den += __shfl_xor(den, 1); den += __shfl_xor(den, 2);
    __syncthreads();
    if (q < tokens) {
        const float inv = 1.f / den;
        for (int c = part * 16; c < part * 16 + 16; ++c) {
            float s = 0.f;
            for (int k = 0; k < tokens; ++k) s += sw[q][k] * sv[k][c];
            out[((size_t)n * tokens + q) * C + head * 64 + c] = (T)(s * inv);
        }
    }
}

template <typename T>
__global__ void prep_input_kernel(const float* __restrict__ x, T* __restrict__ xin, int N, int C, int HW, int cstride, float scale, int ones_idx) {
    size_t i = (size_t)blockIdx.x * blockDim.x + threadIdx.x;
    if (i >= (size_t)N * HW) return;
    int n = (int)(i / HW), p = (int)(i % HW);
    for (int c = 0; c < C; ++c) xin[i * cstride + c] = mul_then_cast<T>(x[((size_t)n * C + c) * HW + p], scale);
    xin[i * cstride + ones_idx] = (T)1.f;
}
template <typename T>
__global__ void write_cond_img_kernel(const float* __restrict__ img, T* __restrict__ xin, int N, int Cc, int HW, int cstride, int c0) {
    size_t i = (size_t)blockIdx.x * blockDim.x + threadIdx.x;
    if (i >= (size_t)N * HW) return;
    int n = (int)(i / HW), p = (int)(i % HW);
    for (int c = 0; c < Cc; ++c) xin[i * cstride + c0 + c] = (T)img[((size_t)n * Cc + c) * HW + p];
}

__global__ void unpack_output_kernel(const float* __restrict__ F, float* __restrict__ y, int N, int C, int HW, int fstride, float scale) {
    size_t i = (size_t)blockIdx.x * blockDim.x + threadIdx.x;
    if (i >= (size_t)N * HW) return;
    int n = (int)(i / HW), p = (int)(i % HW);
    for (int c = 0; c < C; ++c) y[((size_t)n * C + c) * HW + p] = F[i * fstride + c] * scale;
}

template <typename T>
__global__ void dpm_step_kernel(float* __restrict__ x, float* __restrict__ m1, const float* __restrict__ F, T* __restrict__ xin,
                                int N, int C, int HW, int fstride, int cstride, SchedCoef k, const float* __restrict__ Fg, float gscale,
                                T* __restrict__ xin2, float* __restrict__ m2) {
    size_t i = (size_t)blockIdx.x * blockDim.x + threadIdx.x;
    if (i >= (size_t)N * HW) return;
    int n = (int)(i / HW), p = (int)(i % HW);
    for (int c = 0; c < C; ++c) {
        size_t xi = ((size_t)n * C + c) * HW + p;
        float xs = x[xi];
        float f = F[i * fstride + c];
        if (Fg) { const float g = Fg[i * fstride + c]; f = g + gscale * (f - g); }
        float xn, m0;
        const float m1v = (k.order == 1 && !m2) ? 0.f : m1[xi];
        dpm_update(k, xs, f, m1v, k.order == 3 ? m2[xi] : 0.f, xn, m0);
        x[xi] = xn;
        if (m2) m2[xi] = m1v;
        m1[xi] = m0;
        if (!k.last) {
            const T xs_next = mul_then_cast<T>(xn, k.c_in_next);
            xin[i * cstride + c] = xs_next;
            if (xin2) xin2[i * cstride + c] = xs_next;
        }
    }
}

template <typename T>
__global__ void consistency_pre_kernel(const float* __restrict__ sample, const float* __restrict__ z, float* __restrict__ xt, T* __restrict__ xin,
                                       int N, int C, int HW, int cstride, float cos_t, float sin_t, float sigma_data, int ones_idx) {
    size_t i = (size_t)blockIdx.x * blockDim.x + threadIdx.x;
    if (i >= (size_t)N * HW) return;
    int n = (int)(i / HW), p = (int)(i % HW);
    for (int c = 0; c < C; ++c) {
        size_t xi = ((size_t)n * C + c) * HW + p;
        float v = cos_t * sample[xi] + sin_t * (z[xi] * sigma_data);
        xt[xi] = v;
        xin[i * cstride + c] = (T)(v / sigma_data);
    }
    xin[i * cstride + ones_idx] = (T)1.f;
}
__global__ void consistency_post_kernel(const float* __restrict__ xt, const float* __restrict__ F, float* __restrict__ out, int N, int C, int HW,
                                        int fstride, float cos_t, float sin_t, float sigma_data) {
    size_t i = (size_t)blockIdx.x * blockDim.x + threadIdx.x;
    if (i >= (size_t)N * HW) return;
    int n = (int)(i / HW), p = (int)(i % HW);
    for (int c = 0; c < C; ++c) {
        size_t xi = ((size_t)n * C + c) * HW + p;
        float pred = -F[i * fstride + c];
        out[xi] = cos_t * xt[xi] - sin_t * sigma_data * pred;
    }
}

__global__ void ddim_cfg_step_kernel(const float* __restrict__ x, const float* __restrict__ uncond, const float* __restrict__ cond, float* __restrict__ out, size_t n,
                                     float g, float sqrt_one_minus_at, float sqrt_at, float sqrt_aprev, float sqrt_one_minus_aprev) {
    const size_t i = (size_t)blockIdx.x * blockDim.x + threadIdx.x;
    if (i >= n) return;
    const float u = uncond[i], e = u + g * (cond[i] - u);
    const float x0 = (x[i] - sqrt_one_minus_at * e) / sqrt_at;
    out[i] = sqrt_aprev * x0 + sqrt_one_minus_aprev * e;
}

#define PCG_MULT 6364136223846793005ULL
#define PCG_INC 1442695040888963407ULL

__device__ __forceinline__ void lcg_jump(uint64_t n, uint64_t& mul, uint64_t& add) {
    uint64_t cm = PCG_MULT, ca = PCG_INC;
    mul = 1; add = 0;
    while (n) {
        if (n & 1) { mul *= cm; add = add * cm + ca; }
        ca = (cm + 1) * ca; cm *= cm; n >>= 1;
    }
}
__device__ __forceinline__ uint32_t pcg_out(uint64_t s) {
    uint32_t x = (uint32_t)(((s >> 18) ^ s) >> 27), rot = (uint32_t)(s >> 59);
    return (x >> rot) | (x << ((32u - rot) & 31u));
}

__global__ __launch_bounds__(256) void noise_tiles_kernel(const uint64_t* __restrict__ seeds, float* __restrict__ out, int64_t n) {
    constexpr int PPT = 8, NTH = 256, R = PPT * NTH;
    __shared__ int s_scan[NTH];
    __shared__ int s_base;
    const int tid = threadIdx.x;
    float* o = out + (size_t)blockIdx.x * n;
    uint64_t jm, ja, rm, ra;
    lcg_jump((uint64_t)(2 * PPT) * tid, jm, ja);
    lcg_jump((uint64_t)(2 * R), rm, ra);
    uint64_t state = seeds[blockIdx.x] * jm + ja;
    if (tid == 0) s_base = 0;
    __syncthreads();
    const double inv = 1.0 / 4294967296.0;
    while (true) {
        const int base = s_base;
        if (base >= n) break;
        float v1o[PPT], v2o[PPT];
        unsigned accept = 0;
        uint64_t s = state;
#pragma unroll
        for (int j = 0; j < PPT; ++j) {
            s = s * PCG_MULT + PCG_INC; uint32_t u1 = pcg_out(s);
            s = s * PCG_MULT + PCG_INC; uint32_t u2 = pcg_out(s);
            double v1 = 2.0 * ((double)u1 + 1.0) * inv - 1.0;
            double v2 = 2.0 * ((double)u2 + 1.0) * inv - 1.0;
            double r = v1 * v1 + v2 * v2;
            if (r > 0.0 && r < 1.0) {
                double f = sqrt(-2.0 * log(r) / r);
                v1o[j] = (float)(v1 * f); v2o[j] = (float)(v2 * f);
                accept |= 1u << j;
            }
        }
        state = state * rm + ra;
        const int cnt = __popc(accept);
        s_scan[tid] = cnt;
        __syncthreads();
        for (int off = 1; off < NTH; off <<= 1) {
            int v = (tid >= off) ? s_scan[tid - off] : 0;
            __syncthreads();
            s_scan[tid] += v;
            __syncthreads();
        }
        int64_t pos = base + 2 * (int64_t)(s_scan[tid] - cnt);
        const int total = s_scan[NTH - 1];
#pragma unroll
        for (int j = 0; j < PPT; ++j) {
            if (accept & (1u << j)) {
                if (pos < n) o[pos] = v1o[j];
                if (pos + 1 < n) o[pos + 1] = v2o[j];
                pos += 2;
            }
        }
        __syncthreads();
        if (tid == 0) s_base = base + 2 * total;
        __syncthreads();
    }
}

__global__ void noise_gather_kernel(const float* __restrict__ tiles, const int* __restrict__ tile_index, const int* __restrict__ origins,
                                    float* __restrict__ out, int C, int h, int w, int tile_h, int tile_w, float scale) {
    const int win = blockIdx.y;
    const int i = blockIdx.x * blockDim.x + threadIdx.x;
    if (i >= C * h * w) return;
    const int x = i % w, y = (i / w) % h, c = i / (w * h);
    const int gy = origins[2 * win] + y, gx = origins[2 * win + 1] + x;
    auto fdiv = [](int a, int b) { int q = a / b; return (a % b != 0 && ((a < 0) != (b < 0))) ? q - 1 : q; };
    const int ty = fdiv(gy, tile_h), tx = fdiv(gx, tile_w);
    const int ty0 = fdiv(origins[2 * win], tile_h), tx0 = fdiv(origins[2 * win + 1], tile_w);
    const int slot = tile_index[win * 4 + (ty - ty0) * 2 + (tx - tx0)];
    const int yy = gy - ty * tile_h, xx = gx - tx * tile_w;
    out[(size_t)win * C * h * w + i] = tiles[((size_t)slot * C + c) * tile_h * tile_w + yy * tile_w + xx] * scale;
}

__global__ void blend_gather_kernel(const float* __restrict__ x, const float* __restrict__ wwin, float* __restrict__ canvas, int C, int Hc, int Wc,
                                    int size, const int* __restrict__ rowmap, const int* __restrict__ colmap, const int* __restrict__ row_start,
                                    const int* __restrict__ col_start, const int* __restrict__ tile_of, int n_wcols, int accumulate) {
    const int i = blockIdx.x * blockDim.x + threadIdx.x;
    if (i >= Hc * Wc) return;
    const int y = i / Wc, xq = i % Wc;
    float acc[8];
    for (int c = 0; c <= C; ++c) acc[c] = accumulate ? canvas[(size_t)c * Hc * Wc + i] : 0.f;
    for (int a = 0; a < 4; ++a) {
        const int ic = rowmap[y * 4 + a];
        if (ic < 0) continue;
        for (int b = 0; b < 4; ++b) {
            const int jc = colmap[xq * 4 + b];
            if (jc < 0) continue;
            const int slot = tile_of[ic * n_wcols + jc];
            if (slot < 0) continue;
            const int ly = y - row_start[ic], lx = xq - col_start[jc];
            const float w = wwin[ly * size + lx];
            for (int c = 0; c < C; ++c) acc[c] = __builtin_fmaf(x[(((size_t)slot * C + c) * size + ly) * size + lx], w, acc[c]);
            acc[C] += w;
        }
    }
    for (int c = 0; c <= C; ++c) canvas[(size_t)c * Hc * Wc + i] = acc[c];
}

__global__ void regions_gather_kernel(const float* const* __restrict__ wins, const int* __restrict__ desc, int maxk, const float* __restrict__ wwin,
                                      float* __restrict__ out, int C, int h, int w, int size) {
    const int r = blockIdx.y, i = blockIdx.x * blockDim.x + threadIdx.x;
    if (i >= h * w) return;
    const int y = i / w, xq = i % w;
    float acc[8];
    for (int c = 0; c <= C; ++c) acc[c] = 0.f;
    const int* d = desc + (size_t)r * maxk * 3;
    for (int k = 0; k < maxk; ++k) {
        const int slot = d[k * 3];
        if (slot < 0) break;
        const int ly = y - d[k * 3 + 1], lx = xq - d[k * 3 + 2];
        if (ly < 0 || ly >= size || lx < 0 || lx >= size) continue;
        const float wt = wwin[ly * size + lx];
        const float* x = wins[slot];
        for (int c = 0; c < C; ++c) acc[c] = __builtin_fmaf(x[((size_t)c * size + ly) * size + lx], wt, acc[c]);
        acc[C] += wt;
    }
    float* o = out + (size_t)r * (C + 1) * h * w;
    for (int c = 0; c <= C; ++c) o[(size_t)c * h * w + i] = acc[c];
}

__global__ void blend_normalize_kernel(const float* __restrict__ canvas, float* __restrict__ out, int C, int HW, float scale) {
    const int i = blockIdx.x * blockDim.x + threadIdx.x;
    if (i >= HW) return;
    const float wsum = canvas[(size_t)C * HW + i];
    for (int c = 0; c < C; ++c) out[(size_t)c * HW + i] = canvas[(size_t)c * HW + i] / wsum * scale;
}

__global__ void window_extract_kernel(const float* __restrict__ img, float* __restrict__ tiles, const int* __restrict__ origins, int C, int Hc, int Wc, int size) {
    const int win = blockIdx.y;
    const int i = blockIdx.x * blockDim.x + threadIdx.x;
    if (i >= C * size * size) return;
    const int x = i % size, y = (i / size) % size, c = i / (size * size);
    tiles[(size_t)win * C * size * size + i] = img[((size_t)c * Hc + origins[2 * win] + y) * Wc + origins[2 * win + 1] + x];
}

template __global__ void attn_kernel<float>(const float*, float*, int, int);
template __global__ void attn_kernel<__bf16>(const __bf16*, __bf16*, int, int);
template __global__ void attn_kernel<_Float16>(const _Float16*, _Float16*, int, int);
template __global__ void prep_input_kernel<float>(const float*, float*, int, int, int, int, float, int);
template __global__ void prep_input_kernel<__bf16>(const float*, __bf16*, int, int, int, int, float, int);
template __global__ void prep_input_kernel<_Float16>(const float*, _Float16*, int, int, int, int, float, int);
template __global__ void write_cond_img_kernel<float>(const float*, float*, int, int, int, int, int);
template __global__ void write_cond_img_kernel<__bf16>(const float*, __bf16*, int, int, int, int, int);
template __global__ void write_cond_img_kernel<_Float16>(const float*, _Float16*, int, int, int, int, int);
template __global__ void dpm_step_kernel<float>(float*, float*, const float*, float*, int, int, int, int, int, SchedCoef, const float*, float, float*, float*);
template __global__ void dpm_step_kernel<__bf16>(float*, float*, const float*, __bf16*, int, int, int, int, int, SchedCoef, const float*, float, __bf16*, float*);
template __global__ void dpm_step_kernel<_Float16>(float*, float*, const float*, _Float16*, int, int, int, int, int, SchedCoef, const float*, float, _Float16*, float*);
template __global__ void consistency_pre_kernel<float>(const float*, const float*, float*, float*, int, int, int, int, float, float, float, int);
template __global__ void consistency_pre_kernel<__bf16>(const float*, const float*, float*, __bf16*, int, int, int, int, float, float, float, int);
template __global__ void consistency_pre_kernel<_Float16>(const float*, const float*, float*, _Float16*, int, int, int, int, float, float, float, int);

}
```

terrain_diffusion_amd/engine.py:

```python
import ctypes as C

import numpy as np
import torch

from ._lib import lib, check

_engines = {}


class Engine:

    def __init__(self, device_id=0):
        self._h = C.c_void_p()
        check(lib().td_engine_create(int(device_id), C.byref(self._h)))
        self.device_id = int(device_id)
        self._async = False

    def set_async(self, on):
        self.set_option("async", 1 if on else 0)

    def set_option(self, key, value):
        check(lib().td_engine_set_option(self._h, key.encode(), int(value)))
        if key == "async":
            self._async = bool(int(value))

    def synchronize(self):
        check(lib().td_engine_synchronize(self._h))

    def profile_read(self, reset=True):
        a, b, c, d = C.c_double(), C.c_int64(), C.c_double(), C.c_int64()
        check(lib().td_engine_profile_read(self._h, C.byref(a), C.byref(b), C.byref(c), C.byref(d), int(reset)))
        return a.value, b.value, c.value, d.value

    def profile_read_glds(self, reset=True):
        a, b, c = C.c_double(), C.c_double(), C.c_int64()
        check(lib().td_engine_profile_read_glds(self._h, C.byref(a), C.byref(b), C.byref(c), int(reset)))
        return a.value, b.value, c.value

    def profile_ops(self):
        buf = C.create_string_buffer(1 << 20)
        check(lib().td_engine_profile_dump(self._h, buf, len(buf)))
        rows = [l.split("\t") for l in buf.value.decode().splitlines() if l]
        return [(r[0], float(r[1]), int(r[2])) for r in rows]

    @property
    def stream(self):
        return lib().td_engine_stream(self._h)

    def set_stream(self, stream=None):
        h = getattr(stream, "cuda_stream", stream)
        if stream is not None and not h:
            raise ValueError("the legacy default (NULL) stream cannot carry the engine's captured graphs: create a torch.cuda.Stream()")
        check(lib().td_engine_set_stream(self._h, C.c_void_p(int(h)) if h else None))
        if h:
            _SHARED_STREAM[self.device_id] = int(h)
        else:
            _SHARED_STREAM.pop(self.device_id, None)

    def on_stream(self, stream, asynchronous=True):
        eng = self

        class _Ctx:
            def __enter__(self_):
                self_.prev_handle = _SHARED_STREAM.get(eng.device_id)
                self_.prev_async = eng._async
                self_.tctx = None
                if isinstance(stream, torch.cuda.Stream):
                    stream.wait_stream(torch.cuda.current_stream(stream.device))
                    self_.tctx = torch.cuda.stream(stream)
                    self_.tctx.__enter__()
                try:
                    eng.set_stream(stream)
                    eng.set_async(asynchronous)
                except BaseException:
                    if self_.tctx is not None:
                        self_.tctx.__exit__(None, None, None)
                    raise
                return eng

            def __exit__(self_, *exc):
                eng.set_async(False)
                eng.set_stream(self_.prev_handle)
                eng.set_async(self_.prev_async)
                if self_.tctx is not None:
                    self_.tctx.__exit__(*exc)
                    torch.cuda.current_stream(stream.device).wait_stream(stream)
                return False
        return _Ctx()

    def close(self):
        if self._h:
            lib().td_engine_destroy(self._h)
            self._h = C.c_void_p()


def get_engine(device=None) -> Engine:
    if device is None:
        idx = 0
    elif isinstance(device, int):
        idx = device
    else:
        d = torch.device(device)
        if d.type != "cuda":
            raise RuntimeError("terrain_diffusion_amd runs on MI355X only (device must be 'cuda[:i]'); there is no CPU fallback")
        idx = d.index or 0
    if idx not in _engines:
        _engines[idx] = Engine(idx)
    return _engines[idx]


def dpm_coefs(sigmas, sigma_data, solver_order=2, lower_order_final=True):
    s = np.ascontiguousarray(np.asarray(sigmas, dtype=np.float32).reshape(-1))
    out = np.zeros((s.size - 1, 13), np.float32)
    check(lib().td_dpm_coefs(C.c_void_p(s.ctypes.data), s.size - 1, float(sigma_data), int(solver_order), int(bool(lower_order_final)), C.c_void_p(out.ctypes.data)))
    return out


_SHARED_STREAM = {}


def engine_on_current_stream(device) -> bool:
    d = torch.device(device)
    idx = d.index if d.index is not None else torch.cuda.current_device()
    return _SHARED_STREAM.get(idx) == torch.cuda.current_stream(d).cuda_stream


def ptr(t):
    if t is None:
        return None
    if isinstance(t, np.ndarray):
        assert t.flags["C_CONTIGUOUS"]
        return C.c_void_p(t.ctypes.data)
    assert t.is_contiguous()
    if t.is_cuda:
        cs = torch.cuda.current_stream(t.device)
        if _SHARED_STREAM.get(t.device.index if t.device.index is not None else torch.cuda.current_device()) != cs.cuda_stream:
            cs.synchronize()
    return C.c_void_p(t.data_ptr())


def f32(t, device=None):
    t = torch.as_tensor(t)
    t = t.to(dtype=torch.float32)
    if device is not None:
        t = t.to(device)
    return t.contiguous()
```

terrain_diffusion_amd/parallel.py:

```python
import math

import torch
import torch.distributed as dist


from .geometry import tile_starts as _tile_starts


def mesh_shape(world, n_rows, n_cols):
    best = None
    for pr in range(1, world + 1):
        if world % pr:
            continue
        pc = world // pr
        if pr > n_rows or pc > n_cols:
            continue
        score = abs(math.log((n_rows / pr) / (n_cols / pc)))
        if best is None or score < best[0]:
            best = (score, pr, pc)
    if best is None:
        raise ValueError(f"cannot place {world} ranks on a {n_rows}x{n_cols} window grid")
    return best[1], best[2]


def _cuts(n, parts):
    return [(i * n) // parts for i in range(parts + 1)]


class ShardPlan:

    def __init__(self, H, W, tile_size, world, stride=None, extended=False):
        self.H, self.W, self.size, self.world = H, W, tile_size, world
        self.extended = bool(extended)
        stride = stride or tile_size // 2
        self.stride = stride
        self.h_starts, self.w_starts = _tile_starts(H, tile_size, stride), _tile_starts(W, tile_size, stride)
        nr, nc = len(self.h_starts), len(self.w_starts)
        self.pr, self.pc = mesh_shape(world, nr, nc)
        self.row_cuts, self.col_cuts = _cuts(nr, self.pr), _cuts(nc, self.pc)
        self.owner = {}
        self.windows = [[] for _ in range(world)]
        for br in range(self.pr):
            for bc in range(self.pc):
                r = br * self.pc + bc
                for ic in range(self.row_cuts[br], self.row_cuts[br + 1]):
                    for jc in range(self.col_cuts[bc], self.col_cuts[bc + 1]):
                        self.owner[(ic, jc)] = r
                        self.windows[r].append((ic, jc))
        self.regions = []
        for br in range(self.pr):
            for bc in range(self.pc):
                y0 = self.h_starts[self.row_cuts[br]] if br > 0 else 0
                y1 = self.h_starts[self.row_cuts[br + 1]] if br + 1 < self.pr else H
                x0 = self.w_starts[self.col_cuts[bc]] if bc > 0 else 0
                x1 = self.w_starts[self.col_cuts[bc + 1]] if bc + 1 < self.pc else W
                if extended:
                    y1 = self.h_starts[self.row_cuts[br + 1] - 1] + tile_size
                    x1 = self.w_starts[self.col_cuts[bc + 1] - 1] + tile_size
                    y0, x0 = self.h_starts[self.row_cuts[br]], self.w_starts[self.col_cuts[bc]]
                self.regions.append((y0, min(y1, H), x0, min(x1, W)))
        self.needed = []
        for r, (y0, y1, x0, x1) in enumerate(self.regions):
            need = [(ic, jc) for ic, hs in enumerate(self.h_starts) for jc, ws in enumerate(self.w_starts)
                    if hs < y1 and hs + tile_size > y0 and ws < x1 and ws + tile_size > x0]
            self.needed.append(need)
        self.sends = {(s, d): [w for w in self.needed[d] if self.owner[w] == s] for s in range(world) for d in range(world) if s != d}
        self.sends = {k: v for k, v in self.sends.items() if v}

    def seam_bytes(self, channels=5):
        return {k: len(v) * channels * self.size * self.size * 4 for k, v in self.sends.items()}


def exchange_windows(plan: ShardPlan, rank, my_tiles, group=None, seam_comm=None):
    if seam_comm is not None:
        if seam_comm.rank != rank or seam_comm.world != plan.world:
            raise ValueError(f"seam_comm is rank {seam_comm.rank} of {seam_comm.world}, the exchange is for rank {rank} of {plan.world}")
        return seam_comm.exchange_windows(plan, my_tiles.contiguous())
    local_index = {w: i for i, w in enumerate(plan.windows[rank])}
    have = {w: my_tiles[local_index[w]] for w in plan.needed[rank] if plan.owner[w] == rank}
    ops, recv_bufs = [], {}
    host_stage = my_tiles.is_cuda and dist.get_backend(group) == "gloo"
    xdev = torch.device("cpu") if host_stage else my_tiles.device
    for (s, d), wins in sorted(plan.sends.items()):
        if s == rank:
            buf = torch.stack([my_tiles[local_index[w]] for w in wins]).contiguous().to(xdev)
            ops.append(dist.P2POp(dist.isend, buf, d, group))
        elif d == rank:
            buf = torch.empty((len(wins),) + tuple(my_tiles.shape[1:]), dtype=my_tiles.dtype, device=xdev)
            recv_bufs[s] = (buf, wins)
            ops.append(dist.P2POp(dist.irecv, buf, s, group))
    if ops:
        for req in dist.batch_isend_irecv(ops):
            req.wait()
        if my_tiles.is_cuda:
            from .engine import engine_on_current_stream
            if not engine_on_current_stream(my_tiles.device):
                torch.cuda.current_stream(my_tiles.device).synchronize()
    for s, (buf, wins) in recv_bufs.items():
        if host_stage:
            buf = buf.to(my_tiles.device)
        for i, w in enumerate(wins):
            have[w] = buf[i]
    return have


_EXCHANGE_STREAMS = {}


def _engine_stream(model):
    import contextlib
    dev = torch.device(getattr(model, "device", "cpu"))
    if dev.type != "cuda":
        return contextlib.nullcontext()
    idx = dev.index if dev.index is not None else torch.cuda.current_device()
    from .engine import engine_on_current_stream
    if engine_on_current_stream(dev):
        return contextlib.nullcontext()
    if idx not in _EXCHANGE_STREAMS:
        _EXCHANGE_STREAMS[idx] = torch.cuda.Stream(device=idx)
    return model.engine.on_stream(_EXCHANGE_STREAMS[idx], asynchronous=False)


def blend_region(plan: ShardPlan, rank, have, blend_fn, normalize_fn, channels, scale):
    y0, y1, x0, x1 = plan.regions[rank]
    wins = sorted(have)
    tiles = torch.stack([have[w] for w in wins]).contiguous()
    canvas = torch.zeros((channels + 1, y1 - y0, x1 - x0), dtype=torch.float32, device=tiles.device)
    blend_fn(canvas, tiles, wins, [h - y0 for h in plan.h_starts], [w - x0 for w in plan.w_starts], plan.size)
    return normalize_fn(canvas, scale)


def engine_fns(model, scheduler, plan, cond_inputs, *, cond_means, cond_stds, noise_level, histogram_raw, steps, channels, noise_seed, noise_origin,
               max_batch):
    from . import sampling as _s

    def sample_fn(windows):
        outs = []
        cond = torch.as_tensor(cond_inputs, dtype=torch.float32)
        for b0 in range(0, len(windows), max_batch):
            chunk = windows[b0:b0 + max_batch]
            origins = [(noise_origin[0] + plan.h_starts[ic], noise_origin[1] + plan.w_starts[jc]) for ic, jc in chunk]
            c58 = _s._tile_conditioning(cond, chunk, histogram_raw, cond_means, cond_stds, noise_level)
            outs.append(_s.sample_independent_tiles(model, scheduler, origins, c58, steps=steps, tile_size=plan.size, channels=channels,
                                                    noise_seed=noise_seed, return_raw=True))
        return torch.cat(outs)

    def blend_fn(canvas, tiles, wins, hs, ws, size):
        _s.blend_windows(model.engine, canvas, tiles, wins, hs, ws, size, accumulate=False)

    def normalize_fn(canvas, scale):
        return _s.blend_normalize(model.engine, canvas, scale)

    return sample_fn, blend_fn, normalize_fn


def sample_base_diffusion_sharded(model, scheduler, shape, cond_inputs, *, cond_means, cond_stds, noise_level=0.0, histogram_raw, steps=15,
                                  tile_size=64, noise_seed=42 + 5819, noise_origin=(0, 0), max_batch=64, group=None, gather_to=None,
                                  sample_fn=None, blend_fn=None, normalize_fn=None, stats=None, seam_comm=None, _on_engine_stream=False):
    if sample_fn is None and model is not None and not _on_engine_stream:
        with _engine_stream(model):
            return sample_base_diffusion_sharded(model, scheduler, shape, cond_inputs, cond_means=cond_means, cond_stds=cond_stds, noise_level=noise_level,
                                                 histogram_raw=histogram_raw, steps=steps, tile_size=tile_size, noise_seed=noise_seed, noise_origin=noise_origin,
                                                 max_batch=max_batch, group=group, gather_to=gather_to, stats=stats, seam_comm=seam_comm, _on_engine_stream=True)
    B, C_, H, W = shape
    assert B == 1
    rank = dist.get_rank(group) if dist.is_initialized() else 0
    world = dist.get_world_size(group) if dist.is_initialized() else 1
    plan = ShardPlan(H, W, tile_size, world)
    sd = float(scheduler.config.sigma_data)
    if sample_fn is None:
        sample_fn, blend_fn, normalize_fn = engine_fns(model, scheduler, plan, cond_inputs, cond_means=cond_means, cond_stds=cond_stds, noise_level=noise_level,
                                                       histogram_raw=histogram_raw, steps=steps, channels=C_, noise_seed=noise_seed, noise_origin=noise_origin,
                                                       max_batch=max_batch)
    my_tiles = sample_fn(plan.windows[rank])
    if stats is not None:
        import time
        if my_tiles.is_cuda:
            torch.cuda.synchronize(my_tiles.device)
        t0 = time.perf_counter()
    have = exchange_windows(plan, rank, my_tiles, group, seam_comm) if world > 1 else {w: my_tiles[i] for i, w in enumerate(plan.windows[rank])}
    if stats is not None:
        if my_tiles.is_cuda:
            torch.cuda.synchronize(my_tiles.device)
        sb = plan.seam_bytes(C_)
        stats["exchange_s"] = stats.get("exchange_s", 0.0) + (time.perf_counter() - t0)
        stats["seam_bytes_sent"] = sum(v for (s_, d_), v in sb.items() if s_ == rank)
        stats["seam_bytes_received"] = sum(v for (s_, d_), v in sb.items() if d_ == rank)
        stats["seam_bytes_total"] = sum(sb.values())
        stats["mesh"] = [plan.pr, plan.pc]
        stats["windows_this_rank"] = len(plan.windows[rank])
    region = blend_region(plan, rank, have, blend_fn, normalize_fn, C_, 1.0 / sd)
    if gather_to is None:
        return region, plan.regions[rank]
    if world == 1:
        return region[None]
    if rank == gather_to:
        full = torch.empty((C_, H, W), dtype=torch.float32, device=region.device)
        for r, (y0, y1, x0, x1) in enumerate(plan.regions):
            if r == rank:
                full[:, y0:y1, x0:x1] = region
            else:
                buf = torch.empty((C_, y1 - y0, x1 - x0), dtype=torch.float32, device=region.device)
                dist.recv(buf, r, group)
                full[:, y0:y1, x0:x1] = buf
        return full[None]
    dist.send(region.contiguous(), gather_to, group)
    return None


def consistency_engine_fns(model, plan, cond_inputs, *, cond_means, cond_stds, noise_level, histogram_raw, channels, noise_seed, noise_origin, max_batch, sigma_data):
    from . import sampling as _s
    from . import noise as _noise
    from ._lib import lib, check
    from .engine import ptr
    dev = model.device

    def step_fn(windows, k, t, prev_tiles):
        cond = torch.as_tensor(cond_inputs, dtype=torch.float32)
        outs = []
        for b0 in range(0, len(windows), max_batch):
            chunk = windows[b0:b0 + max_batch]
            origins = [(noise_origin[0] + plan.h_starts[ic], noise_origin[1] + plan.w_starts[jc]) for ic, jc in chunk]
            z = _noise.gaussian_noise_patches(noise_seed + k, origins, plan.size, plan.size, channels=channels, tile_h=64, tile_w=64, device=dev)
            c58 = _s._tile_conditioning(cond, chunk, histogram_raw, cond_means, cond_stds, noise_level).to(dev).contiguous()
            prev = None if prev_tiles is None else prev_tiles[b0:b0 + max_batch].contiguous()
            out = torch.empty_like(z)
            check(lib().td_sample_consistency(model._h, z.shape[0], plan.size, plan.size, float(t), float(sigma_data), ptr(prev), ptr(z), ptr(c58), ptr(out)))
            outs.append(out)
        return torch.cat(outs)

    def blend_fn(canvas, tiles, wins, hs, ws, size):
        _s.blend_windows(model.engine, canvas, tiles, wins, hs, ws, size, accumulate=False)

    def normalize_fn(canvas, scale):
        return _s.blend_normalize(model.engine, canvas, scale)

    return step_fn, blend_fn, normalize_fn


def sample_base_consistency_sharded(model, scheduler, shape, cond_inputs, *, cond_means, cond_stds, noise_level=0.0, histogram_raw, intermediate_t=0.0,
                                    tile_size=64, noise_seed=42 + 5819, noise_origin=(0, 0), max_batch=64, group=None, gather_to=None,
                                    step_fn=None, blend_fn=None, normalize_fn=None, stats=None, seam_comm=None, _on_engine_stream=False):
    if step_fn is None and model is not None and not _on_engine_stream:
        with _engine_stream(model):
            return sample_base_consistency_sharded(model, scheduler, shape, cond_inputs, cond_means=cond_means, cond_stds=cond_stds, noise_level=noise_level,
                                                   histogram_raw=histogram_raw, intermediate_t=intermediate_t, tile_size=tile_size, noise_seed=noise_seed,
                                                   noise_origin=noise_origin, max_batch=max_batch, group=group, gather_to=gather_to, stats=stats,
                                                   seam_comm=seam_comm, _on_engine_stream=True)
    B, C_, H, W = shape
    assert B == 1
    rank = dist.get_rank(group) if dist.is_initialized() else 0
    world = dist.get_world_size(group) if dist.is_initialized() else 1
    own, ext = ShardPlan(H, W, tile_size, world), ShardPlan(H, W, tile_size, world, extended=True)
    sd = float(scheduler.config.sigma_data)
    t0 = float(torch.atan(torch.tensor(float(scheduler.config.sigma_max), dtype=torch.float32) / sd))
    t_scalars = (t0, float(torch.tensor(intermediate_t, dtype=torch.float32))) if intermediate_t > 0 else (t0,)
    if step_fn is None:
        step_fn, blend_fn, normalize_fn = consistency_engine_fns(model, own, cond_inputs, cond_means=cond_means, cond_stds=cond_stds, noise_level=noise_level,
                                                                 histogram_raw=histogram_raw, channels=C_, noise_seed=noise_seed, noise_origin=noise_origin,
                                                                 max_batch=max_batch, sigma_data=sd)
    mine = own.windows[rank]
    prev_tiles, region = None, None
    for k, t in enumerate(t_scalars):
        last = k == len(t_scalars) - 1
        plan = own if last else ext
        out = step_fn(mine, k, t, prev_tiles)
        have = exchange_windows(plan, rank, out, group, seam_comm) if world > 1 else {w: out[i] for i, w in enumerate(mine)}
        if stats is not None:
            stats["exchanges"] = stats.get("exchanges", 0) + (1 if world > 1 else 0)
            stats["seam_bytes_total"] = stats.get("seam_bytes_total", 0) + sum(plan.seam_bytes(C_).values())
        region = blend_region(plan, rank, have, blend_fn, normalize_fn, C_, (1.0 / sd) if last else 1.0)
        if not last:
            y0, _, x0, _ = ext.regions[rank]
            prev_tiles = torch.stack([region[:, own.h_starts[ic] - y0:own.h_starts[ic] - y0 + tile_size, own.w_starts[jc] - x0:own.w_starts[jc] - x0 + tile_size]
                                      for ic, jc in mine]).contiguous()
    if gather_to is None:
        return region, own.regions[rank]
    if world == 1:
        return region[None]
    if rank == gather_to:
        full = torch.empty((C_, H, W), dtype=torch.float32, device=region.device)
        for r, (y0, y1, x0, x1) in enumerate(own.regions):
            if r == rank:
                full[:, y0:y1, x0:x1] = region
            else:
                buf = torch.empty((C_, y1 - y0, x1 - x0), dtype=torch.float32, device=region.device)
                dist.recv(buf, r, group)
                full[:, y0:y1, x0:x1] = buf
        return full[None]
    dist.send(region.contiguous(), gather_to, group)
    return None


def shard_requests(boxes, world=None, rank=None):
    world = (dist.get_world_size() if dist.is_initialized() else 1) if world is None else world
    rank = (dist.get_rank() if dist.is_initialized() else 0) if rank is None else rank

    def z(ci, cj):
        ci, cj = int(ci) + (1 << 30), int(cj) + (1 << 30)
        v = 0
        for b in range(31):
            v |= ((ci >> b) & 1) << (2 * b + 1) | ((cj >> b) & 1) << (2 * b)
        return v
    order = sorted(range(len(boxes)), key=lambda k: z((boxes[k][0] + boxes[k][2]) // 2, (boxes[k][1] + boxes[k][3]) // 2))
    lo, hi = (rank * len(order)) // world, ((rank + 1) * len(order)) // world
    return [(k, boxes[k]) for k in order[lo:hi]]
```

terrain_diffusion_amd/sampling.py:

```python
import ctypes as C
import math

import numpy as np
import torch

from ._lib import lib, check
from .engine import ptr
from . import noise as _noise


from .geometry import tile_starts as _tile_starts


def _linear_weight_window(size, device="cuda", dtype=torch.float32):
    from .engine import get_engine
    eng = get_engine(device)
    out = torch.empty((size, size), dtype=torch.float32, device=torch.device("cuda", eng.device_id))
    check(lib().td_linear_weight_window(eng._h, size, ptr(out)))
    return out[None, None]


def _process_cond_img(cond_img, histogram_raw, cond_means, cond_stds, noise_level=0.0):
    cond_img = torch.as_tensor(cond_img, dtype=torch.float32).cpu()
    means = torch.as_tensor(cond_means, dtype=torch.float32).view(1, -1, 1, 1)
    stds = torch.as_tensor(cond_stds, dtype=torch.float32).view(1, -1, 1, 1)
    cond_img = (cond_img - means) / stds
    cm = torch.as_tensor(cond_means, dtype=torch.float32).flatten()
    cond_img[0:1] = torch.nan_to_num(cond_img[0:1], nan=float(cm[0]))
    cond_img[1:2] = torch.nan_to_num(cond_img[1:2], nan=float(cm[1]))
    B = cond_img.shape[0]
    nl = (torch.as_tensor(noise_level, dtype=torch.float32) - 0.5) * np.sqrt(12)
    hist = torch.as_tensor(histogram_raw, dtype=torch.float32)
    clim = cond_img[:, 2:6, 1:3, 1:3].mean(dim=(2, 3))
    nan_mask = torch.isnan(clim)
    if bool(nan_mask.any()):
        from .noise import standard_normal
        cnt = int(nan_mask.sum())
        clim[nan_mask] = torch.from_numpy(standard_normal(9999 + cnt, (cnt,), dtype=np.float32))
    parts = [cond_img[:, 0:1].flatten(1), cond_img[:, 1:2].flatten(1), clim.flatten(1),
             cond_img[:, 6:7].flatten(1), hist.view(-1, hist.shape[-1]).expand(B, -1), nl.view(-1, 1).expand(B, 1)]
    n = len(parts)
    Cc = math.sqrt(sum(p.shape[1] for p in parts) / (n * (1.0 / n) ** 2))
    return torch.cat([p * (Cc / math.sqrt(p.shape[1]) * (1.0 / n)) for p in parts], dim=1).float()


def process_latent_conditioning(cond_img, histogram_raw, cond_means, cond_stds, noise_level=0.0, *, seed, seed_offset=0):
    from .noise import standard_normal
    cond_img = torch.as_tensor(cond_img, dtype=torch.float32)
    dev = cond_img.device
    cond_means = torch.as_tensor(cond_means, dtype=torch.float32)
    cond_stds = torch.as_tensor(cond_stds, dtype=torch.float32)
    cond_img = (cond_img - cond_means.view(1, -1, 1, 1).to(dev)) / cond_stds.view(1, -1, 1, 1).to(dev)
    cond_img[0:1] = cond_img[0:1].nan_to_num(float(cond_means[0]))
    cond_img[1:2] = cond_img[1:2].nan_to_num(float(cond_means[1]))
    clim = cond_img[:, 2:6, 1:3, 1:3].mean(dim=(2, 3))
    nan_mask = torch.isnan(clim)
    cnt = int(nan_mask.sum())
    if cnt > 0:
        clim[nan_mask] = torch.from_numpy(standard_normal(seed + 9999 + seed_offset, (cnt,), dtype=np.float32)).to(dev)
    B = cond_img.shape[0]
    nl = ((torch.as_tensor(noise_level, dtype=torch.float32) - 0.5) * np.sqrt(12)).to(dev)
    hist = torch.as_tensor(histogram_raw, dtype=torch.float32).to(dev)
    parts = [cond_img[:, 0:1].flatten(1), cond_img[:, 1:2].flatten(1), clim.flatten(1), cond_img[:, 6:7].flatten(1),
             hist.view(-1, hist.shape[-1]).expand(B, -1), nl.view(-1, 1).expand(B, 1)]
    n = len(parts)
    Cc = math.sqrt(sum(p.shape[1] for p in parts) / (n * (1.0 / n) ** 2))
    return torch.cat([p * (Cc / math.sqrt(p.shape[1]) * (1.0 / n)) for p in parts], dim=1).float()


_DEV_CONST = {}


def _dev_const(t, dev):
    t = torch.as_tensor(t, dtype=torch.float32)
    if t.device == dev or t.is_cuda:
        return t.to(dev)
    key = (t.numpy().tobytes(), tuple(t.shape), str(dev))
    v = _DEV_CONST.get(key)
    if v is None:
        if len(_DEV_CONST) > 64:
            _DEV_CONST.clear()
        v = _DEV_CONST[key] = t.to(dev)
    return v


def process_latent_conditioning_windows(cond_imgs, histogram_raw, cond_means, cond_stds, noise_level=0.0):
    x = torch.as_tensor(cond_imgs, dtype=torch.float32)
    dev = x.device
    cond_means = torch.as_tensor(cond_means, dtype=torch.float32)
    cond_stds = torch.as_tensor(cond_stds, dtype=torch.float32)
    x = ((x - _dev_const(cond_means.view(1, -1, 1, 1), dev)) / _dev_const(cond_stds.view(1, -1, 1, 1), dev)).nan_to_num(float(cond_means[0]))
    clim = x[:, 2:6, 1:3, 1:3].mean(dim=(2, 3))
    B = x.shape[0]
    nl = (torch.as_tensor(noise_level, dtype=torch.float32) - 0.5) * np.sqrt(12)
    nl = torch.full((1, 1), float(nl), dtype=torch.float32, device=dev) if nl.numel() == 1 and not nl.is_cuda else nl.to(dev)
    hist = _dev_const(histogram_raw, dev)
    parts = [x[:, 0:1].flatten(1), x[:, 1:2].flatten(1), clim.flatten(1), x[:, 6:7].flatten(1), hist.view(-1, hist.shape[-1]).expand(B, -1), nl.view(-1, 1).expand(B, 1)]
    n = len(parts)
    Cc = math.sqrt(sum(p.shape[1] for p in parts) / (n * (1.0 / n) ** 2))
    return torch.cat([p * (Cc / math.sqrt(p.shape[1]) * (1.0 / n)) for p in parts], dim=1).float()


def _tile_conditioning(cond_inputs, tiles, histogram_raw, cond_means, cond_stds, noise_level):
    if cond_inputs.ndim == 4:
        return torch.cat([_process_cond_img(cond_inputs[..., ic:ic + 4, jc:jc + 4], histogram_raw, cond_means, cond_stds, noise_level)
                          for ic, jc in tiles], dim=0)
    return torch.as_tensor(cond_inputs, dtype=torch.float32).view(1, -1).expand(len(tiles), -1).contiguous()


def blend_windows(engine, canvas, tiles, tile_idx, h_starts, w_starts, size, accumulate=True):
    C_, Hc, Wc = canvas.shape[0] - 1, canvas.shape[1], canvas.shape[2]
    rs = np.asarray(h_starts, dtype=np.int32)
    cs = np.asarray(w_starts, dtype=np.int32)
    wi = np.asarray([t[0] for t in tile_idx], dtype=np.int32)
    wj = np.asarray([t[1] for t in tile_idx], dtype=np.int32)
    check(lib().td_blend_windows(engine._h, ptr(canvas), C_, Hc, Wc, size, len(rs), C.c_void_p(rs.ctypes.data), len(cs), C.c_void_p(cs.ctypes.data),
                                 len(wi), C.c_void_p(wi.ctypes.data), C.c_void_p(wj.ctypes.data), ptr(tiles), int(accumulate)))
    return canvas


def blend_normalize(engine, canvas, scale=1.0):
    C_, Hc, Wc = canvas.shape[0] - 1, canvas.shape[1], canvas.shape[2]
    out = torch.empty((C_, Hc, Wc), dtype=torch.float32, device=canvas.device)
    check(lib().td_blend_normalize(engine._h, ptr(canvas), C_, Hc, Wc, float(scale), ptr(out)))
    return out


@torch.no_grad()
def sample_tiles_edm(model, scheduler, x, cond, steps, cond_img=None, guide_model=None, guidance_scale=1.0):
    scheduler.set_timesteps(steps)
    sig = scheduler.sigmas.to(torch.float32).cpu().contiguous()
    model.engine.set_option("solver_order", int(getattr(scheduler.config, "solver_order", 2)))
    model.engine.set_option("lower_order_final", int(bool(getattr(scheduler.config, "lower_order_final", True))))
    n, _, H, W = x.shape
    cimg = 0 if cond_img is None else cond_img.shape[1]
    if guide_model is not None and guidance_scale != 1.0:
        if cond_img is not None:
            raise NotImplementedError("autoguidance with conditioning-image channels")
        check(lib().td_sample_edm_guided(model._h, guide_model._h, float(guidance_scale), n, H, W, steps, ptr(sig), float(scheduler.config.sigma_data), ptr(cond), ptr(x)))
        return x
    check(lib().td_sample_edm_img(model._h, n, H, W, steps, ptr(sig), float(scheduler.config.sigma_data), ptr(cond), ptr(cond_img), cimg, ptr(x)))
    return x


@torch.no_grad()
def consistency_step(model, t, sigma_data, sample, z, cond=None, cond_img=None):
    n, _, H, W = z.shape
    out = torch.empty_like(z)
    cimg = 0 if cond_img is None else cond_img.shape[1]
    check(lib().td_sample_consistency_img(model._h, n, H, W, float(t), float(sigma_data), ptr(sample), ptr(z), ptr(cond), ptr(cond_img), cimg, ptr(out)))
    return out


@torch.no_grad()
def sample_base_diffusion(model, scheduler, shape, cond_inputs, *, cond_means, cond_stds, noise_level=0.0, histogram_raw, dtype=torch.float32,
                          steps=15, guide_model=None, guidance_scale=1.0, generator=None, tile_size=None, weight_window_fn=None,
                          noise_seed=42 + 5819, noise_origin=(0, 0), tiles=None, max_batch=64, return_canvas=False, return_windows=False):
    if weight_window_fn is not None:
        raise NotImplementedError("custom weight windows")
    B, C_, H, W = shape
    if B != 1:
        raise NotImplementedError("B == 1 (one canvas) per call")
    eng, dev = model.engine, model.device
    sd = float(scheduler.config.sigma_data)
    scheduler.set_timesteps(steps)
    sigma0 = float(scheduler.sigmas[0])
    if tile_size is None:
        tile_size_eff, h_starts, w_starts = None, [0], [0]
        th, tw = H, W
    else:
        stride = tile_size // 2
        h_starts, w_starts = _tile_starts(H, tile_size, stride), _tile_starts(W, tile_size, stride)
        th = tw = tile_size
    cond_inputs = torch.as_tensor(cond_inputs, dtype=torch.float32)
    if tile_size is not None and cond_inputs.ndim == 1 and len(h_starts) * len(w_starts) > 1:
        raise ValueError(f"cond_inputs must be a tensor image for tiled sampling. Cond inputs must have width {len(w_starts)+3} and height {len(h_starts)+3}.")
    if cond_inputs.ndim == 4:
        assert cond_inputs.shape[-1] == len(w_starts) + 3 and cond_inputs.shape[-2] == len(h_starts) + 3
    all_tiles = [(ic, jc) for ic in range(len(h_starts)) for jc in range(len(w_starts))]
    run = all_tiles if tiles is None else [t for t in all_tiles if t in set(tiles)]
    canvas = torch.zeros((C_ + 1, H, W), dtype=torch.float32, device=dev)
    windows = {}
    for b0 in range(0, len(run), max_batch):
        chunk = run[b0:b0 + max_batch]
        origins = [(noise_origin[0] + h_starts[ic], noise_origin[1] + w_starts[jc]) for ic, jc in chunk]
        nth, ntw = max(64, th), max(64, tw)
        x = _noise.gaussian_noise_patches(noise_seed, origins, th, tw, channels=C_, tile_h=nth, tile_w=ntw, scale=sigma0, device=dev)
        cond = _tile_conditioning(cond_inputs, chunk, histogram_raw, cond_means, cond_stds, noise_level).to(dev).contiguous()
        sample_tiles_edm(model, scheduler, x, cond, steps, guide_model=guide_model, guidance_scale=guidance_scale)
        if tile_size is None:
            return x
        if return_windows:
            windows.update({t: x[k].clone() for k, t in enumerate(chunk)})
        blend_windows(eng, canvas, x, chunk, h_starts, w_starts, tile_size, accumulate=True)
    out = canvas if return_canvas else blend_normalize(eng, canvas, 1.0 / sd)[None]
    return (out, windows) if return_windows else out


@torch.no_grad()
def sample_independent_tiles(model, scheduler, origins, cond, *, steps=20, tile_size=64, channels=5, noise_seed=42 + 5819, return_raw=False):
    eng, dev = model.engine, model.device
    sd = float(scheduler.config.sigma_data)
    scheduler.set_timesteps(steps)
    n = len(origins)
    x = _noise.gaussian_noise_patches(noise_seed, origins, tile_size, tile_size, channels=channels, tile_h=64, tile_w=64,
                                      scale=float(scheduler.sigmas[0]), device=dev)
    cond = torch.as_tensor(cond, dtype=torch.float32).to(dev).contiguous()
    sample_tiles_edm(model, scheduler, x, cond, steps)
    if return_raw:
        return x
    canvas = torch.empty((channels + 1, n * tile_size, tile_size), dtype=torch.float32, device=dev)
    blend_windows(eng, canvas, x, [(i, 0) for i in range(n)], [i * tile_size for i in range(n)], [0], tile_size, accumulate=False)
    out = blend_normalize(eng, canvas, 1.0 / sd)
    return out.view(channels, n, tile_size, tile_size).permute(1, 0, 2, 3)


@torch.no_grad()
def sample_base_consistency(model, scheduler, shape, cond_inputs, *, cond_means, cond_stds, noise_level=0.0, histogram_raw, intermediate_t=0.0,
                            dtype=torch.float32, generator=None, tile_size=None, weight_window_fn=None, noise=None,
                            noise_seed=42 + 5819, noise_origin=(0, 0), max_batch=64):
    B, C_, H, W = shape
    if B != 1 or tile_size is None or weight_window_fn is not None:
        raise NotImplementedError
    eng, dev = model.engine, model.device
    sd = float(scheduler.config.sigma_data)
    init_t = math.atan(float(scheduler.config.sigma_max) / sd) if noise is None else None
    sigma0 = scheduler.sigmas[0] if noise is not None else None
    t0 = float(torch.atan(torch.tensor(scheduler.config.sigma_max, dtype=torch.float32) / sd))
    t_scalars = (t0, float(torch.tensor(intermediate_t, dtype=torch.float32))) if intermediate_t > 0 else (t0,)
    stride = tile_size // 2
    h_starts, w_starts = _tile_starts(H, tile_size, stride), _tile_starts(W, tile_size, stride)
    cond_inputs = torch.as_tensor(cond_inputs, dtype=torch.float32)
    tiles = [(ic, jc) for ic in range(len(h_starts)) for jc in range(len(w_starts))]
    origins = [(h_starts[ic], w_starts[jc]) for ic, jc in tiles]
    cond_all = _tile_conditioning(cond_inputs, tiles, histogram_raw, cond_means, cond_stds, noise_level).to(dev).contiguous()
    sample = None
    for k, t in enumerate(t_scalars):
        canvas = torch.zeros((C_ + 1, H, W), dtype=torch.float32, device=dev)
        for b0 in range(0, len(tiles), max_batch):
            sl = slice(b0, b0 + max_batch)
            if noise is None:
                z = _noise.gaussian_noise_patches(noise_seed + k, [(noise_origin[0] + y, noise_origin[1] + x) for y, x in origins[sl]], tile_size, tile_size,
                                                  channels=C_, tile_h=64, tile_w=64, device=dev)
            else:
                z = torch.stack([torch.as_tensor(noise[k])[0, :, y:y + tile_size, x:x + tile_size] for y, x in origins[sl]]).to(dev, torch.float32).contiguous()
            prev = None
            if sample is not None:
                prev = torch.stack([sample[:, y:y + tile_size, x:x + tile_size] for y, x in origins[sl]]).contiguous()
            out = torch.empty_like(z)
            cond = cond_all[sl].contiguous()
            check(lib().td_sample_consistency(model._h, z.shape[0], tile_size, tile_size, float(t), sd, ptr(prev), ptr(z), ptr(cond), ptr(out)))
            blend_windows(eng, canvas, out, tiles[sl], h_starts, w_starts, tile_size, accumulate=True)
        sample = blend_normalize(eng, canvas, 1.0)
    return (sample / sd)[None]


def _cond_tiles(cond_img, h, w, device):
    cond_img = torch.as_tensor(cond_img).to(device=device, dtype=torch.float32)
    if tuple(cond_img.shape[-2:]) != (h, w):
        cond_img = torch.nn.functional.interpolate(cond_img, size=(h, w), mode="nearest")
    return cond_img.contiguous()


def _blend_batch(eng, tiles, b, n_tiles, tile_idx, h_starts, w_starts, tile_size, h, w, scale):
    C_ = tiles.shape[1]
    outs = []
    for k in range(b):
        canvas = torch.zeros((C_ + 1, h, w), dtype=torch.float32, device=tiles.device)
        blend_windows(eng, canvas, tiles[k::b].contiguous(), tile_idx, h_starts, w_starts, tile_size, accumulate=False)
        outs.append(blend_normalize(eng, canvas, scale))
    return torch.stack(outs)


def _tile_geometry(h, w, tile_size, tile_stride, default):
    tile_size = default if tile_size is None else int(tile_size)
    tile_stride = tile_size if tile_stride is None else int(tile_stride)
    h_starts, w_starts = _tile_starts(h, tile_size, tile_stride), _tile_starts(w, tile_size, tile_stride)
    tile_idx = [(ic, jc) for ic in range(len(h_starts)) for jc in range(len(w_starts))]
    return tile_size, h_starts, w_starts, tile_idx


@torch.no_grad()
def sample_decoder_diffusion_tiled(model, scheduler, cond_img, noise, tile_size=None, tile_stride=None, *, num_steps=None, guidance_model=None,
                                   guidance_scale=1.0, score_scaling=1.0, weight_window_fn=None, max_batch=64):
    if weight_window_fn is not None or score_scaling != 1.0:
        raise NotImplementedError("custom weight windows / score scaling")
    if guidance_model is not None and guidance_scale != 1.0:
        raise NotImplementedError("autoguidance with conditioning-image channels")
    if num_steps is not None:
        scheduler.set_timesteps(num_steps)
    steps = len(scheduler.timesteps)
    eng, dev = model.engine, model.device
    noise = torch.as_tensor(noise).to(device=dev, dtype=torch.float32)
    b, c, h, w = noise.shape
    cond_img = _cond_tiles(cond_img, h, w, dev)
    T, h_starts, w_starts, tile_idx = _tile_geometry(h, w, tile_size, tile_stride, min(h, w))
    outs = []
    jobs = [(i0, j0) for i0 in h_starts for j0 in w_starts]
    per = max(1, max_batch // b)
    for a in range(0, len(jobs), per):
        chunk = jobs[a:a + per]
        x = torch.cat([noise[:, :, i0:i0 + T, j0:j0 + T] for i0, j0 in chunk]).contiguous()
        ci = torch.cat([cond_img[:, :, i0:i0 + T, j0:j0 + T] for i0, j0 in chunk]).contiguous()
        outs.append(sample_tiles_edm(model, scheduler, x, None, steps, cond_img=ci))
    return _blend_batch(eng, torch.cat(outs), b, len(jobs), tile_idx, h_starts, w_starts, T, h, w, 1.0)


@torch.no_grad()
def sample_decoder_consistency_tiled(model, scheduler, cond_img, noise, tile_size=None, tile_stride=None, *, intermediate_t=None, weight_window_fn=None,
                                     max_batch=64):
    if weight_window_fn is not None:
        raise NotImplementedError("custom weight windows")
    eng, dev = model.engine, model.device
    noise = torch.as_tensor(noise).to(device=dev, dtype=torch.float32)
    b, c, h, w = noise.shape
    cond_img = _cond_tiles(cond_img, h, w, dev)
    sd = float(scheduler.config.sigma_data)
    init_t = float(torch.atan(torch.as_tensor(float(scheduler.sigmas[0]) / sd, dtype=torch.float32)))
    if intermediate_t is None:
        extra = []
    elif torch.is_tensor(intermediate_t):
        extra = [float(t) for t in intermediate_t.flatten().to(torch.float32)]
    elif isinstance(intermediate_t, (list, tuple)):
        extra = [float(torch.tensor(t, dtype=torch.float32)) for t in intermediate_t]
    else:
        extra = [float(torch.tensor(float(intermediate_t), dtype=torch.float32))]
    T, h_starts, w_starts, tile_idx = _tile_geometry(h, w, tile_size, tile_stride, min(h, w))
    jobs = [(i0, j0) for i0 in h_starts for j0 in w_starts]
    per = max(1, max_batch // b)
    outs = []
    for a in range(0, len(jobs), per):
        chunk = jobs[a:a + per]
        z = torch.cat([noise[:, :, i0:i0 + T, j0:j0 + T] for i0, j0 in chunk]).contiguous()
        ci = torch.cat([cond_img[:, :, i0:i0 + T, j0:j0 + T] for i0, j0 in chunk]).contiguous()
        sample = None
        for t in [init_t] + extra:
            sample = consistency_step(model, t, sd, sample, z, cond=None, cond_img=ci)
        outs.append(sample)
    return _blend_batch(eng, torch.cat(outs), b, len(jobs), tile_idx, h_starts, w_starts, T, h, w, 1.0 / sd)


@torch.no_grad()
def sample_coarse_tiled(model, scheduler, cond_img, cond_snr, *, steps=15, tile_size=None, tile_stride=None, weight_window_fn=None, generator=None,
                        dtype=torch.float32, cond_noise=None, init_noise=None, noise_seed=42, max_batch=64):
    if weight_window_fn is not None:
        raise NotImplementedError("custom weight windows")
    eng, dev = model.engine, model.device
    cond_img = torch.as_tensor(cond_img).to(device=dev, dtype=torch.float32)
    assert cond_img.ndim == 4, "cond_img must be [B, C, H, W]"
    b, c_cond, h, w = cond_img.shape
    T, h_starts, w_starts, tile_idx = _tile_geometry(h, w, tile_size, tile_stride, w)
    if h < T or w < T:
        raise ValueError(f"sample_coarse_tiled: the conditioning image ({h} x {w}) is smaller than the tile ({T} x {T}); pass tile_size <= min(h, w)")
    c_out = int(model.config["out_channels"])
    snr = torch.as_tensor(cond_snr, dtype=torch.float32)
    t_cond = torch.atan(snr)
    cond_vals = torch.log(torch.tan(t_cond) / 8.0)
    cond_inputs = [v.reshape(-1) for v in cond_vals.reshape(-1, cond_vals.shape[-1]).transpose(0, 1)]
    tc = t_cond.reshape(1, -1, 1, 1).to(dev)
    if cond_noise is None:
        cond_noise = torch.from_numpy(_noise.standard_normal(noise_seed, tuple(cond_img.shape)))
    cond_img = (torch.cos(tc) * cond_img + torch.sin(tc) * torch.as_tensor(cond_noise).to(dev, torch.float32)).contiguous()
    scheduler.set_timesteps(int(steps))
    sd = float(scheduler.config.sigma_data)
    sigma0 = float(scheduler.sigmas[0])
    jobs = [(i0, j0) for i0 in h_starts for j0 in w_starts]
    per = max(1, max_batch // b)
    outs = []
    for a in range(0, len(jobs), per):
        chunk = list(enumerate(jobs))[a:a + per]
        xs = []
        for k, (i0, j0) in chunk:
            z = init_noise[k] if init_noise is not None else torch.from_numpy(_noise.standard_normal(noise_seed + 1 + k, (b, c_out, T, T)))
            xs.append(torch.as_tensor(z).to(dev, torch.float32) * sigma0)
        x = torch.cat(xs).contiguous()
        ci = torch.cat([cond_img[:, :, i0:i0 + T, j0:j0 + T] for _, (i0, j0) in chunk]).contiguous()
        n = x.shape[0]
        cond = model.cond_rows([v if v.numel() == 1 else v.repeat(len(chunk)) for v in cond_inputs], n, dev)
        sample_tiles_edm(model, scheduler, x, cond, int(steps), cond_img=ci)
        outs.append(x)
    return _blend_batch(eng, torch.cat(outs), b, len(jobs), tile_idx, h_starts, w_starts, T, h, w, 1.0 / sd)
```

Measured before the change: 20.91 MP/s.

## Fuse noise, conditioning, EDM sampling and blending into one grid-batch native call

Adds a td_sample_grid_batch entry point that runs noise generation, per-tile conditioning rows (now built by a GPU kernel via td_cond_rows), the EDM sampler and window blending in a single native call on the engine stream. It replaces several Python-level round trips, host-side conditioning assembly and separate synchronizing calls per chunk. The aim is to cut host overhead and intermediate syncs between stages. It is gated by a new grid_fused option that defaults to on, and the new path must match the old conditioning math exactly.

After: 21.32 MP/s (median of 6 runs). 1.02x the previous value.

```diff
diff --git a/include/td_engine.h b/include/td_engine.h
--- a/include/td_engine.h
+++ b/include/td_engine.h
@@ -41,6 +41,7 @@
 void* td_engine_stream(td_engine* e);
 int td_engine_set_stream(td_engine* e, void* hip_stream);
 int td_engine_set_option(td_engine* e, const char* key, int64_t value);
+int64_t td_engine_get_option(td_engine* e, const char* key, int64_t dflt);
 
 int td_engine_profile_read(td_engine* e, double* conv_ms, int64_t* conv_launches, double* other_ms, int64_t* other_launches, int reset);
 
@@ -79,6 +80,36 @@
 int td_sample_consistency_img(td_unet* u, int n, int H, int W, float t, float sigma_data, const float* sample, const float* z,
                               const float* cond, const float* cond_img, int cimg_channels, float* out);
 
+int td_cond_rows(td_engine* e, const float* grid, int grid_rows, int grid_cols, int n, const int32_t* pos_host, const float* means_host,
+                 const float* stds_host, const float* hist_host, int n_hist, float noise_level, float* out);
+
+typedef struct td_grid_batch {
+    uint64_t noise_seed;
+    int32_t n, H, W, tile_h, tile_w;
+    float noise_scale;
+    const int64_t* origins_host;
+    const float* cond_rows;
+    const float* cond_grid;
+    int32_t grid_rows, grid_cols;
+    const int32_t* cond_pos_host;
+    const float* cond_means_host;
+    const float* cond_stds_host;
+    const float* hist_host;
+    int32_t n_hist;
+    float noise_level;
+    int32_t n_steps;
+    float sigma_data;
+    const float* sigmas_host;
+    float* canvas;
+    int32_t Hc, Wc, size, n_rows, n_cols, accumulate;
+    const int32_t* row_starts_host;
+    const int32_t* col_starts_host;
+    const int32_t* wi_host;
+    const int32_t* wj_host;
+    float* windows_out;
+} td_grid_batch;
+int td_sample_grid_batch(td_unet* u, const td_grid_batch* batch);
+
 int td_blend_windows(td_engine* e, float* canvas, int C, int Hc, int Wc, int size, int n_rows, const int32_t* row_starts_host,
                      int n_cols, const int32_t* col_starts_host, int n_tiles, const int32_t* wi_host, const int32_t* wj_host,
                      const float* tiles, int accumulate);
diff --git a/terrain_diffusion_amd/_lib.py b/terrain_diffusion_amd/_lib.py
--- a/terrain_diffusion_amd/_lib.py
+++ b/terrain_diffusion_amd/_lib.py
@@ -45,6 +45,17 @@
 
 
 _P = C.c_void_p
+
+
+class GridBatch(C.Structure):
+    _fields_ = [("noise_seed", C.c_uint64), ("n", C.c_int32), ("H", C.c_int32), ("W", C.c_int32), ("tile_h", C.c_int32), ("tile_w", C.c_int32),
+                ("noise_scale", C.c_float), ("origins_host", _P), ("cond_rows", _P), ("cond_grid", _P), ("grid_rows", C.c_int32), ("grid_cols", C.c_int32),
+                ("cond_pos_host", _P), ("cond_means_host", _P), ("cond_stds_host", _P), ("hist_host", _P), ("n_hist", C.c_int32), ("noise_level", C.c_float),
+                ("n_steps", C.c_int32), ("sigma_data", C.c_float), ("sigmas_host", _P), ("canvas", _P), ("Hc", C.c_int32), ("Wc", C.c_int32),
+                ("size", C.c_int32), ("n_rows", C.c_int32), ("n_cols", C.c_int32), ("accumulate", C.c_int32), ("row_starts_host", _P),
+                ("col_starts_host", _P), ("wi_host", _P), ("wj_host", _P), ("windows_out", _P)]
+
+
 _SIGS = {
     "td_last_error": (C.c_char_p, []),
     "td_version": (C.c_int, []),
@@ -55,6 +66,7 @@
     "td_engine_stream": (_P, [_P]),
     "td_engine_set_stream": (C.c_int, [_P, _P]),
     "td_engine_set_option": (C.c_int, [_P, C.c_char_p, C.c_int64]),
+    "td_engine_get_option": (C.c_int64, [_P, C.c_char_p, C.c_int64]),
     "td_engine_profile_read": (C.c_int, [_P, C.POINTER(C.c_double), C.POINTER(C.c_int64), C.POINTER(C.c_double), C.POINTER(C.c_int64), C.c_int]),
     "td_engine_profile_read_glds": (C.c_int, [_P, C.POINTER(C.c_double), C.POINTER(C.c_double), C.POINTER(C.c_int64), C.c_int]),
     "td_engine_profile_dump": (C.c_int, [_P, C.c_char_p, C.c_int64]),
@@ -72,6 +84,8 @@
     "td_tile_seed": (C.c_uint64, [C.c_uint64, C.c_int64, C.c_int64]),
     "td_standard_normal": (C.c_int, [_P, C.c_uint64, C.c_int64, _P]),
     "td_noise_patches": (C.c_int, [_P, C.c_uint64, C.c_int, _P, C.c_int, C.c_int, C.c_int, C.c_int, C.c_int, C.c_float, _P]),
+    "td_cond_rows": (C.c_int, [_P, _P, C.c_int, C.c_int, C.c_int, _P, _P, _P, _P, C.c_int, C.c_float, _P]),
+    "td_sample_grid_batch": (C.c_int, [_P, C.POINTER(GridBatch)]),
     "td_sample_edm": (C.c_int, [_P, C.c_int, C.c_int, C.c_int, C.c_int, _P, C.c_float, _P, _P]),
     "td_sample_edm_guided": (C.c_int, [_P, _P, C.c_float, C.c_int, C.c_int, C.c_int, C.c_int, _P, C.c_float, _P, _P]),
     "td_sample_consistency": (C.c_int, [_P, C.c_int, C.c_int, C.c_int, C.c_float, C.c_float, _P, _P, _P, _P]),
diff --git a/terrain_diffusion_amd/csrc/engine.hip b/terrain_diffusion_amd/csrc/engine.hip
--- a/terrain_diffusion_amd/csrc/engine.hip
+++ b/terrain_diffusion_amd/csrc/engine.hip
@@ -1150,7 +1150,7 @@
 }
 static const char* const kKnownOptions[] = {
     "async", "batch_invariant", "fuse_solver", "graph", "lower_order_final", "profile", "solver_order", "dual_stream", "dual_stream_min_batch", "sampler_stop_after",
-    "plan_cache_mb", "plan_cache_max",
+    "plan_cache_mb", "plan_cache_max", "grid_fused",
     "attn_mfma", "bn128_min_wgs", "glds", "glds_bn", "glds_bn64", "glds_dma1x1", "glds_min_wgs", "glds_round_aware", "glds_small_max_groups",
     "glds_splitk", "glds_splitk_from_groups", "glds_splitk_max", "glds_splitk_min_groups", "glds_tiny", "glds_variant", "glds_wide", "glds_wide_min_wgs", "glds_wide_tail", "glds_wide_persist", "fewcout",
     "producer_act", "s16", "s16_min_wgs", "sb", "sb_m4", "sb_max_glds_wgs", "sb_mt", "sb_nt", "sb_order", "sb_splitk", "sb_splitk_max", "sb_splitk_wgs", "sb_target_wgs", "splitk",
@@ -1163,6 +1163,8 @@
     e->opt[key] = value;
     return TD_OK;
 }
+
+int64_t td_engine_get_option(td_engine* e, const char* key, int64_t dflt) { return (e && key) ? e->option(key, dflt) : dflt; }
 
 int td_engine_profile_read(td_engine* e, double* conv_ms, int64_t* conv_launches, double* other_ms, int64_t* other_launches, int reset) {
     if (conv_ms) *conv_ms = e->prof_conv_ms;
@@ -1520,18 +1522,15 @@
     return TD_OK;
 }
 
-static int sample_edm_impl(td_unet* u, td_unet* guide, float gscale, int n, int H, int W, int n_steps, const float* sigmas_host, float sigma_data,
-                           const float* cond, const float* cond_img, int cimg, float* x) {
+static int sample_edm_enqueue(td_unet* u, td_unet* guide, float gscale, int n, int H, int W, int n_steps, const float* sigmas_host, float sigma_data,
+                              const float* cond, const float* cond_img, int cimg, float* x, std::vector<Buf>& hold) {
     td_engine* e = u->eng;
-    DevGuard dg_(e->device);
-    std::vector<Buf> hold;
     const bool dual = e->stream2 && e->option("dual_stream", 1) != 0 && n >= std::max<int64_t>(2, e->option("dual_stream_min_batch", 32));
     const bool concurrent = e->option("profile", 0) == 0;
-    const bool all_dev = is_device_ptr(x) && (!cond || is_device_ptr(cond)) && (!cond_img || is_device_ptr(cond_img));
     if (!dual) {
         int rc = sample_edm_lane(u, guide, gscale, n, H, W, n_steps, sigmas_host, sigma_data, cond, cond_img, cimg, x, 0, hold);
-        if (rc) { (void)hipStreamSynchronize(e->stream); return rc; }
-        return end_call(e, hold, all_dev);
+        if (rc) (void)hipStreamSynchronize(e->stream);
+        return rc;
     }
     const int nA = n / 2, nB = n - nA, C = u->cfg.out_channels;
     const size_t HW = (size_t)H * W;
@@ -1545,6 +1544,17 @@
     }
     if (rc) { (void)hipStreamSynchronize(e->stream); (void)hipStreamSynchronize(e->stream2); return rc; }
     if (concurrent) { HIP_TRY(hipEventRecord(e->ev_join, e->stream2)); HIP_TRY(hipStreamWaitEvent(e->stream, e->ev_join, 0)); }
+    return TD_OK;
+}
+
+static int sample_edm_impl(td_unet* u, td_unet* guide, float gscale, int n, int H, int W, int n_steps, const float* sigmas_host, float sigma_data,
+                           const float* cond, const float* cond_img, int cimg, float* x) {
+    td_engine* e = u->eng;
+    DevGuard dg_(e->device);
+    std::vector<Buf> hold;
+    const bool all_dev = is_device_ptr(x) && (!cond || is_device_ptr(cond)) && (!cond_img || is_device_ptr(cond_img));
+    int rc = sample_edm_enqueue(u, guide, gscale, n, H, W, n_steps, sigmas_host, sigma_data, cond, cond_img, cimg, x, hold);
+    if (rc) return rc;
     return end_call(e, hold, all_dev);
 }
 
@@ -1624,14 +1634,18 @@
 
 static inline int64_t fdiv(int64_t a, int64_t b) { int64_t q = a / b; return (a % b != 0 && ((a < 0) != (b < 0))) ? q - 1 : q; }
 
-int td_noise_patches(td_engine* e, uint64_t base_seed, int n_windows, const int64_t* origins, int h, int w, int channels, int tile_h, int tile_w,
-                     float scale, float* out) {
-    DevGuard dg_(e->device);
-    if (n_windows <= 0) return TD_OK;
+struct NoiseJob {
+    std::vector<uint64_t> seeds;
+    std::vector<int> index, org;
+    Buf dseeds, dtiles, dindex, dorg;
+    int64_t tn = 0;
+};
+static int noise_prepare(td_engine* e, NoiseJob& j, uint64_t base_seed, int n_windows, const int64_t* origins, int h, int w, int channels, int tile_h, int tile_w) {
     if (h > tile_h || w > tile_w) return fail(TD_ERR_UNSUPPORTED, "window larger than the noise tile");
     std::map<std::pair<int64_t, int64_t>, int> slot;
-    std::vector<uint64_t> seeds;
-    std::vector<int> index((size_t)n_windows * 4, 0), org((size_t)n_windows * 2);
+    std::vector<uint64_t>& seeds = j.seeds;
+    std::vector<int>& index = j.index; std::vector<int>& org = j.org;
+    index.assign((size_t)n_windows * 4, 0); org.resize((size_t)n_windows * 2);
     for (int i = 0; i < n_windows; ++i) {
         const int64_t y0 = origins[2 * i], x0 = origins[2 * i + 1];
         org[2 * i] = (int)y0; org[2 * i + 1] = (int)x0;
@@ -1645,21 +1659,35 @@
                 index[(size_t)i * 4 + (ty - ty0) * 2 + (tx - tx0)] = s;
             }
     }
-    const int64_t tn = (int64_t)channels * tile_h * tile_w;
-    Buf dseeds(new DevBuf()), dtiles(new DevBuf()), dindex(new DevBuf()), dorg(new DevBuf());
-    HIP_TRY(dseeds->scratch(e->scratch, seeds.size() * 8)); HIP_TRY(dtiles->scratch(e->scratch, seeds.size() * tn * 4));
-    HIP_TRY(dindex->scratch(e->scratch, index.size() * 4)); HIP_TRY(dorg->scratch(e->scratch, org.size() * 4));
+    j.tn = (int64_t)channels * tile_h * tile_w;
+    j.dseeds.reset(new DevBuf()); j.dtiles.reset(new DevBuf()); j.dindex.reset(new DevBuf()); j.dorg.reset(new DevBuf());
+    HIP_TRY(j.dseeds->scratch(e->scratch, seeds.size() * 8)); HIP_TRY(j.dtiles->scratch(e->scratch, seeds.size() * j.tn * 4));
+    HIP_TRY(j.dindex->scratch(e->scratch, index.size() * 4)); HIP_TRY(j.dorg->scratch(e->scratch, org.size() * 4));
+    int rc;
+    if ((rc = upload(e, j.dseeds->p, seeds.data(), seeds.size() * 8)) || (rc = upload(e, j.dindex->p, index.data(), index.size() * 4)) ||
+        (rc = upload(e, j.dorg->p, org.data(), org.size() * 4))) return rc;
+    return TD_OK;
+}
+static int noise_enqueue(td_engine* e, const NoiseJob& j, int n_windows, int h, int w, int channels, int tile_h, int tile_w, float scale, float* out_dev) {
     hipStream_t st = e->stream;
+    hipLaunchKernelGGL(noise_tiles_kernel, dim3((unsigned)j.seeds.size()), dim3(256), 0, st, (const uint64_t*)j.dseeds->p, (float*)j.dtiles->p, j.tn);
+    hipLaunchKernelGGL(noise_gather_kernel, dim3((channels * h * w + 255) / 256, n_windows), dim3(256), 0, st, (const float*)j.dtiles->p, (const int*)j.dindex->p,
+                       (const int*)j.dorg->p, out_dev, channels, h, w, tile_h, tile_w, scale);
+    HIP_TRY(hipGetLastError());
+    return TD_OK;
+}
+
+int td_noise_patches(td_engine* e, uint64_t base_seed, int n_windows, const int64_t* origins, int h, int w, int channels, int tile_h, int tile_w,
+                     float scale, float* out) {
+    DevGuard dg_(e->device);
+    if (n_windows <= 0) return TD_OK;
+    NoiseJob j;
     int rc;
-    if ((rc = upload(e, dseeds->p, seeds.data(), seeds.size() * 8)) || (rc = upload(e, dindex->p, index.data(), index.size() * 4)) ||
-        (rc = upload(e, dorg->p, org.data(), org.size() * 4))) return rc;
+    if ((rc = noise_prepare(e, j, base_seed, n_windows, origins, h, w, channels, tile_h, tile_w))) return rc;
     std::vector<Buf> hold;
     OutStage os;
     if ((rc = out_device(e, out, (size_t)n_windows * channels * h * w * 4, hold, &os))) return rc;
-    hipLaunchKernelGGL(noise_tiles_kernel, dim3((unsigned)seeds.size()), dim3(256), 0, st, (const uint64_t*)dseeds->p, (float*)dtiles->p, tn);
-    hipLaunchKernelGGL(noise_gather_kernel, dim3((channels * h * w + 255) / 256, n_windows), dim3(256), 0, st, (const float*)dtiles->p, (const int*)dindex->p,
-                       (const int*)dorg->p, (float*)os.dev, channels, h, w, tile_h, tile_w, scale);
-    HIP_TRY(hipGetLastError());
+    if ((rc = noise_enqueue(e, j, n_windows, h, w, channels, tile_h, tile_w, scale, (float*)os.dev))) return rc;
     if ((rc = out_finish(e, os))) return rc;
     return end_call(e, hold, !os.host);
 }
@@ -1686,12 +1714,16 @@
     return TD_OK;
 }
 
-int td_blend_windows(td_engine* e, float* canvas, int C, int Hc, int Wc, int size, int n_rows, const int32_t* row_starts, int n_cols,
-                     const int32_t* col_starts, int n_tiles, const int32_t* wi, const int32_t* wj, const float* tiles, int accumulate) {
-    DevGuard dg_(e->device);
+struct BlendJob {
+    std::vector<int> rowmap, colmap, tile_of;
+    std::vector<float> ww;
+    Buf drow, dcol, drs, dcs, dtof, dww;
+};
+static int blend_prepare(td_engine* e, BlendJob& j, int C, int Hc, int Wc, int size, int n_rows, const int32_t* row_starts, int n_cols, const int32_t* col_starts,
+                         int n_tiles, const int32_t* wi, const int32_t* wj) {
     if (C + 1 > 8) return fail(TD_ERR_UNSUPPORTED, "C+1 must be <= 8");
-    hipStream_t st = e->stream;
-    std::vector<int> rowmap((size_t)Hc * 4, -1), colmap((size_t)Wc * 4, -1), tile_of((size_t)n_rows * n_cols, -1);
+    std::vector<int>& rowmap = j.rowmap; std::vector<int>& colmap = j.colmap; std::vector<int>& tile_of = j.tile_of;
+    rowmap.assign((size_t)Hc * 4, -1); colmap.assign((size_t)Wc * 4, -1); tile_of.assign((size_t)n_rows * n_cols, -1);
     for (int ic = 0; ic < n_rows; ++ic)
         for (int y = std::max(0, row_starts[ic]); y < std::min(Hc, row_starts[ic] + size); ++y) {
             int k = 0;
@@ -1710,18 +1742,32 @@
         if (wi[i] < 0 || wi[i] >= n_rows || wj[i] < 0 || wj[i] >= n_cols) return fail(TD_ERR_ARG, "window index out of range");
         tile_of[(size_t)wi[i] * n_cols + wj[i]] = i;
     }
-    std::vector<float> ww;
-    weight_window_host(size, ww);
+    weight_window_host(size, j.ww);
     auto up = [&](const void* src, size_t bytes, Buf& b) -> int {
         b.reset(new DevBuf());
         HIP_TRY(b->scratch(e->scratch, bytes));
         return upload(e, b->p, src, bytes);
     };
-    Buf drow, dcol, drs, dcs, dtof, dww;
     int rc;
-    if ((rc = up(rowmap.data(), rowmap.size() * 4, drow)) || (rc = up(colmap.data(), colmap.size() * 4, dcol)) || (rc = up(row_starts, (size_t)n_rows * 4, drs)) ||
-        (rc = up(col_starts, (size_t)n_cols * 4, dcs)) || (rc = up(tile_of.data(), tile_of.size() * 4, dtof)) || (rc = up(ww.data(), ww.size() * 4, dww)))
+    if ((rc = up(rowmap.data(), rowmap.size() * 4, j.drow)) || (rc = up(colmap.data(), colmap.size() * 4, j.dcol)) || (rc = up(row_starts, (size_t)n_rows * 4, j.drs)) ||
+        (rc = up(col_starts, (size_t)n_cols * 4, j.dcs)) || (rc = up(tile_of.data(), tile_of.size() * 4, j.dtof)) || (rc = up(j.ww.data(), j.ww.size() * 4, j.dww)))
         return rc;
+    return TD_OK;
+}
+static int blend_enqueue(td_engine* e, const BlendJob& j, float* dcanvas, int C, int Hc, int Wc, int size, int n_cols, const float* dtiles, int accumulate) {
+    hipLaunchKernelGGL(blend_gather_kernel, grid1((size_t)Hc * Wc), dim3(256), 0, e->stream, dtiles, (const float*)j.dww->p, dcanvas, C, Hc, Wc, size,
+                       (const int*)j.drow->p, (const int*)j.dcol->p, (const int*)j.drs->p, (const int*)j.dcs->p, (const int*)j.dtof->p, n_cols, accumulate);
+    HIP_TRY(hipGetLastError());
+    return TD_OK;
+}
+
+int td_blend_windows(td_engine* e, float* canvas, int C, int Hc, int Wc, int size, int n_rows, const int32_t* row_starts, int n_cols,
+                     const int32_t* col_starts, int n_tiles, const int32_t* wi, const int32_t* wj, const float* tiles, int accumulate) {
+    DevGuard dg_(e->device);
+    hipStream_t st = e->stream;
+    BlendJob j;
+    int rc;
+    if ((rc = blend_prepare(e, j, C, Hc, Wc, size, n_rows, row_starts, n_cols, col_starts, n_tiles, wi, wj))) return rc;
     std::vector<Buf> hold;
     const void* dt;
     if ((rc = to_device(e, tiles, (size_t)n_tiles * C * size * size * 4, hold, &dt))) return rc;
@@ -1735,9 +1781,7 @@
         dcanvas = (float*)cstage->p;
         if (accumulate) HIP_TRY(hipMemcpyAsync(dcanvas, canvas, cbytes, hipMemcpyHostToDevice, st));
     }
-    hipLaunchKernelGGL(blend_gather_kernel, grid1((size_t)Hc * Wc), dim3(256), 0, st, (const float*)dt, (const float*)dww->p, dcanvas, C, Hc, Wc, size,
-                       (const int*)drow->p, (const int*)dcol->p, (const int*)drs->p, (const int*)dcs->p, (const int*)dtof->p, n_cols, accumulate);
-    HIP_TRY(hipGetLastError());
+    if ((rc = blend_enqueue(e, j, dcanvas, C, Hc, Wc, size, n_cols, (const float*)dt, accumulate))) return rc;
     if (!cdev) HIP_TRY(hipMemcpyAsync(canvas, dcanvas, cbytes, hipMemcpyDeviceToHost, st));
     return end_call(e, hold, cdev && is_device_ptr(tiles));
 }
@@ -1785,6 +1829,102 @@
     HIP_TRY(hipGetLastError());
     if ((rc = out_finish(e, os))) return rc;
     return end_call(e, hold, !os.host && is_device_ptr(canvas));
+}
+
+struct CondJob {
+    std::vector<int32_t> stage;
+    Buf dstage;
+    const void* dgrid = nullptr;
+    CondRowsParams p;
+};
+static int cond_prepare(td_engine* e, CondJob& j, const float* grid, int R, int Cg, int n, const int32_t* pos, const float* means, const float* stds,
+                        const float* hist, int nh, float noise_level, std::vector<Buf>& hold) {
+    if (!grid || !pos || !means || !stds || (nh > 0 && !hist)) return fail(TD_ERR_ARG, "td_cond_rows: null argument");
+    if (n < 1 || R < 4 || Cg < 4 || nh < 0 || nh > 4096) return fail(TD_ERR_ARG, "td_cond_rows: n >= 1, a grid of at least 4 x 4 cells, 0 <= nh <= 4096");
+    for (int i = 0; i < n; ++i)
+        if (pos[2 * i] < 0 || pos[2 * i] + 4 > R || pos[2 * i + 1] < 0 || pos[2 * i + 1] + 4 > Cg) return fail(TD_ERR_ARG, "td_cond_rows: window position outside the grid");
+    CondRowsParams& p = j.p;
+    for (int c = 0; c < 7; ++c) { p.mean[c] = means[c]; p.stdv[c] = stds[c]; }
+    const int L[6] = {16, 16, 4, 16, nh, 1};
+    const double inv = 1.0 / 6;
+    const double Cc = sqrt((double)(53 + nh) / (6 * pow(inv, 2.0)));
+    for (int k = 0; k < 6; ++k) p.factor[k] = L[k] > 0 ? (float)(Cc / sqrt((double)L[k]) * inv) : 0.f;
+    p.nan_fill = means[0];
+    p.noise_entry = (noise_level - 0.5f) * (float)sqrt(12.0);
+    p.R = R; p.Cg = Cg; p.nh = nh; p.n = n;
+    int rc;
+    if ((rc = to_device(e, grid, (size_t)7 * R * Cg * 4, hold, &j.dgrid))) return rc;
+    j.stage.resize((size_t)2 * n + nh);
+    memcpy(j.stage.data(), pos, (size_t)2 * n * 4);
+    if (nh) memcpy(j.stage.data() + (size_t)2 * n, hist, (size_t)nh * 4);
+    j.dstage.reset(new DevBuf());
+    HIP_TRY(j.dstage->scratch(e->scratch, j.stage.size() * 4));
+    return upload(e, j.dstage->p, j.stage.data(), j.stage.size() * 4);
+}
+static int cond_enqueue(td_engine* e, const CondJob& j, float* out_dev) {
+    const int32_t* d = (const int32_t*)j.dstage->p;
+    hipLaunchKernelGGL(cond_rows_kernel, grid1((size_t)j.p.n * (53 + j.p.nh)), dim3(256), 0, e->stream, (const float*)j.dgrid, (const int*)d,
+                       (const float*)(d + (size_t)2 * j.p.n), out_dev, j.p);
+    HIP_TRY(hipGetLastError());
+    return TD_OK;
+}
+
+int td_cond_rows(td_engine* e, const float* grid, int grid_rows, int grid_cols, int n, const int32_t* pos_host, const float* means_host, const float* stds_host,
+                 const float* hist_host, int n_hist, float noise_level, float* out) {
+    if (!e || !out) return fail(TD_ERR_ARG, "td_cond_rows: null argument");
+    DevGuard dg_(e->device);
+    std::vector<Buf> hold;
+    CondJob j;
+    int rc;
+    if ((rc = cond_prepare(e, j, grid, grid_rows, grid_cols, n, pos_host, means_host, stds_host, hist_host, n_hist, noise_level, hold))) return rc;
+    OutStage os;
+    if ((rc = out_device(e, out, (size_t)n * (53 + n_hist) * 4, hold, &os))) return rc;
+    if ((rc = cond_enqueue(e, j, (float*)os.dev))) return rc;
+    if ((rc = out_finish(e, os))) return rc;
+    return end_call(e, hold, !os.host && is_device_ptr(grid));
+}
+
+int td_sample_grid_batch(td_unet* u, const td_grid_batch* b) {
+    if (!u || !b) return fail(TD_ERR_ARG, "td_sample_grid_batch: null argument");
+    td_engine* e = u->eng;
+    DevGuard dg_(e->device);
+    if (!u->finalized) return fail(TD_ERR_STATE, "finalize first");
+    const int n = b->n, H = b->H, W = b->W, C = u->cfg.out_channels;
+    if (n < 1 || H < 1 || W < 1 || !b->origins_host || !b->sigmas_host || b->n_steps < 1) return fail(TD_ERR_ARG, "td_sample_grid_batch: bad batch description");
+    if (u->cfg.in_channels != C) return fail(TD_ERR_ARG, "td_sample_grid_batch: models with conditioning-image channels take td_sample_edm_img");
+    if (!b->canvas && !b->windows_out) return fail(TD_ERR_ARG, "td_sample_grid_batch: neither a canvas nor a window buffer to write to");
+    if ((b->canvas && !is_device_ptr(b->canvas)) || (b->windows_out && !is_device_ptr(b->windows_out))) return fail(TD_ERR_ARG, "td_sample_grid_batch: canvas and window buffer are device buffers");
+    if (b->canvas && (H != b->size || W != b->size)) return fail(TD_ERR_ARG, "td_sample_grid_batch: the blend takes square windows of `size`");
+    if (u->cond_row_len > 0 && !b->cond_rows && !b->cond_grid) return fail(TD_ERR_ARG, "td_sample_grid_batch: the model takes conditioning rows");
+    if (b->cond_grid && !b->cond_rows && 53 + b->n_hist != u->cond_row_len) return fail(TD_ERR_ARG, "td_sample_grid_batch: 53 + n_hist must equal the model's conditioning row length");
+    std::vector<Buf> hold;
+    NoiseJob nj; CondJob cj; BlendJob bj;
+    int rc;
+    auto bail = [&](int code) { (void)hipStreamSynchronize(e->stream); return code; };
+    if ((rc = noise_prepare(e, nj, b->noise_seed, n, b->origins_host, H, W, C, b->tile_h, b->tile_w))) return bail(rc);
+    const void* drows = nullptr;
+    const bool rows_from_grid = u->cond_row_len > 0 && !b->cond_rows;
+    if (rows_from_grid) {
+        if ((rc = cond_prepare(e, cj, b->cond_grid, b->grid_rows, b->grid_cols, n, b->cond_pos_host, b->cond_means_host, b->cond_stds_host, b->hist_host, b->n_hist,
+                               b->noise_level, hold))) return bail(rc);
+        Buf r(new DevBuf());
+        if (r->scratch(e->scratch, (size_t)n * u->cond_row_len * 4) != hipSuccess) return bail(fail(TD_ERR_HIP, "td_sample_grid_batch: scratch allocation"));
+        drows = r->p;
+        hold.push_back(std::move(r));
+    } else if (u->cond_row_len > 0 && (rc = to_device(e, b->cond_rows, (size_t)n * u->cond_row_len * 4, hold, &drows))) return bail(rc);
+    if (b->canvas && (rc = blend_prepare(e, bj, C, b->Hc, b->Wc, b->size, b->n_rows, b->row_starts_host, b->n_cols, b->col_starts_host, n, b->wi_host, b->wj_host))) return bail(rc);
+    float* x = b->windows_out;
+    if (!x) {
+        Buf xb(new DevBuf());
+        if (xb->scratch(e->scratch, (size_t)n * C * H * W * 4) != hipSuccess) return bail(fail(TD_ERR_HIP, "td_sample_grid_batch: scratch allocation"));
+        x = (float*)xb->p;
+        hold.push_back(std::move(xb));
+    }
+    if ((rc = noise_enqueue(e, nj, n, H, W, C, b->tile_h, b->tile_w, b->noise_scale, x))) return bail(rc);
+    if (rows_from_grid && (rc = cond_enqueue(e, cj, (float*)drows))) return bail(rc);
+    if ((rc = sample_edm_enqueue(u, nullptr, 1.f, n, H, W, b->n_steps, b->sigmas_host, b->sigma_data, (const float*)drows, nullptr, 0, x, hold))) return bail(rc);
+    if (b->canvas && (rc = blend_enqueue(e, bj, b->canvas, C, b->Hc, b->Wc, b->size, b->n_cols, x, b->accumulate))) return bail(rc);
+    return end_call(e, hold, (!b->cond_rows || is_device_ptr(b->cond_rows)) && (!rows_from_grid || is_device_ptr(b->cond_grid)));
 }
 
 int td_resample2d(td_engine* e, const float* in, int C, int Hin, int Win, int Hout, int Wout, const int32_t* iy, const float* wy, int Ky,
diff --git a/terrain_diffusion_amd/csrc/small_kernels.hip b/terrain_diffusion_amd/csrc/small_kernels.hip
--- a/terrain_diffusion_amd/csrc/small_kernels.hip
+++ b/terrain_diffusion_amd/csrc/small_kernels.hip
@@ -443,6 +443,41 @@
     tiles[(size_t)win * C * size * size + i] = img[((size_t)c * Hc + origins[2 * win] + y) * Wc + origins[2 * win + 1] + x];
 }
 
+struct CondRowsParams {
+    float mean[7], stdv[7];
+    float factor[6];
+    float nan_fill;
+    float noise_entry;
+    int R, Cg, nh, n;
+};
+
+__global__ void cond_rows_kernel(const float* __restrict__ grid, const int* __restrict__ pos, const float* __restrict__ hist, float* __restrict__ out, CondRowsParams p) {
+#pragma clang fp contract(off)
+    const int L = 53 + p.nh;
+    const int t = blockIdx.x * blockDim.x + threadIdx.x;
+    if (t >= p.n * L) return;
+    const int win = t / L, k = t % L;
+    const int i0 = pos[2 * win], j0 = pos[2 * win + 1];
+    auto cell = [&](int c, int y, int x) {
+        float v = __fdiv_rn(__fsub_rn(grid[((size_t)c * p.R + i0 + y) * p.Cg + j0 + x], p.mean[c]), p.stdv[c]);
+        if (v != v) v = p.nan_fill;
+        else if (v > 3.402823466e+38f) v = 3.402823466e+38f;
+        else if (v < -3.402823466e+38f) v = -3.402823466e+38f;
+        return v;
+    };
+    float r;
+    if (k < 16) r = __fmul_rn(cell(0, k >> 2, k & 3), p.factor[0]);
+    else if (k < 32) r = __fmul_rn(cell(1, (k - 16) >> 2, k & 3), p.factor[1]);
+    else if (k < 36) {
+        const int c = 2 + (k - 32);
+        const float a = cell(c, 1, 1), b = cell(c, 1, 2), cc = cell(c, 2, 1), d = cell(c, 2, 2);
+        r = __fmul_rn(__fdiv_rn(__fadd_rn(__fadd_rn(a, b), __fadd_rn(cc, d)), 4.f), p.factor[2]);
+    } else if (k < 52) r = __fmul_rn(cell(6, (k - 36) >> 2, k & 3), p.factor[3]);
+    else if (k < 52 + p.nh) r = __fmul_rn(hist[k - 52], p.factor[4]);
+    else r = __fmul_rn(p.noise_entry, p.factor[5]);
+    out[t] = r;
+}
+
 template __global__ void attn_kernel<float>(const float*, float*, int, int);
 template __global__ void attn_kernel<__bf16>(const __bf16*, __bf16*, int, int);
 template __global__ void attn_kernel<_Float16>(const _Float16*, _Float16*, int, int);
diff --git a/terrain_diffusion_amd/engine.py b/terrain_diffusion_amd/engine.py
--- a/terrain_diffusion_amd/engine.py
+++ b/terrain_diffusion_amd/engine.py
@@ -23,6 +23,9 @@
         check(lib().td_engine_set_option(self._h, key.encode(), int(value)))
         if key == "async":
             self._async = bool(int(value))
+
+    def get_option(self, key, default):
+        return int(lib().td_engine_get_option(self._h, key.encode(), int(default)))
 
     def synchronize(self):
         check(lib().td_engine_synchronize(self._h))
diff --git a/terrain_diffusion_amd/parallel.py b/terrain_diffusion_amd/parallel.py
--- a/terrain_diffusion_amd/parallel.py
+++ b/terrain_diffusion_amd/parallel.py
@@ -140,7 +140,7 @@
         for b0 in range(0, len(windows), max_batch):
             chunk = windows[b0:b0 + max_batch]
             origins = [(noise_origin[0] + plan.h_starts[ic], noise_origin[1] + plan.w_starts[jc]) for ic, jc in chunk]
-            c58 = _s._tile_conditioning(cond, chunk, histogram_raw, cond_means, cond_stds, noise_level)
+            c58 = _s.tile_conditioning_rows(model.engine, cond, chunk, histogram_raw, cond_means, cond_stds, noise_level)
             outs.append(_s.sample_independent_tiles(model, scheduler, origins, c58, steps=steps, tile_size=plan.size, channels=channels,
                                                     noise_seed=noise_seed, return_raw=True))
         return torch.cat(outs)
@@ -222,7 +222,7 @@
             chunk = windows[b0:b0 + max_batch]
             origins = [(noise_origin[0] + plan.h_starts[ic], noise_origin[1] + plan.w_starts[jc]) for ic, jc in chunk]
             z = _noise.gaussian_noise_patches(noise_seed + k, origins, plan.size, plan.size, channels=channels, tile_h=64, tile_w=64, device=dev)
-            c58 = _s._tile_conditioning(cond, chunk, histogram_raw, cond_means, cond_stds, noise_level).to(dev).contiguous()
+            c58 = _s.tile_conditioning_rows(model.engine, cond, chunk, histogram_raw, cond_means, cond_stds, noise_level).to(dev).contiguous()
             prev = None if prev_tiles is None else prev_tiles[b0:b0 + max_batch].contiguous()
             out = torch.empty_like(z)
             check(lib().td_sample_consistency(model._h, z.shape[0], plan.size, plan.size, float(t), float(sigma_data), ptr(prev), ptr(z), ptr(c58), ptr(out)))
diff --git a/terrain_diffusion_amd/sampling.py b/terrain_diffusion_amd/sampling.py
--- a/terrain_diffusion_amd/sampling.py
+++ b/terrain_diffusion_amd/sampling.py
@@ -4,7 +4,7 @@
 import numpy as np
 import torch
 
-from ._lib import lib, check
+from ._lib import lib, check, GridBatch
 from .engine import ptr
 from . import noise as _noise
 
@@ -108,6 +108,36 @@
     return torch.as_tensor(cond_inputs, dtype=torch.float32).view(1, -1).expand(len(tiles), -1).contiguous()
 
 
+def _np32(t):
+    return np.ascontiguousarray(torch.as_tensor(t, dtype=torch.float32).detach().cpu().numpy().reshape(-1))
+
+
+def _cond_grid_args(cond_inputs, histogram_raw, cond_means, cond_stds, noise_level):
+    g = torch.as_tensor(cond_inputs)
+    if g.ndim != 4 or g.shape[0] != 1 or g.shape[1] != 7 or g.shape[2] < 4 or g.shape[3] < 4:
+        return None
+    means, stds, hist = _np32(cond_means), _np32(cond_stds), torch.as_tensor(histogram_raw, dtype=torch.float32)
+    nl = torch.as_tensor(noise_level, dtype=torch.float32)
+    if means.size != 7 or stds.size != 7 or hist.numel() != hist.shape[-1] or nl.numel() != 1:
+        return None
+    return g[0].to(torch.float32).contiguous(), means, stds, _np32(hist), float(nl.reshape(()))
+
+
+def cond_rows(engine, cond_inputs, tiles, histogram_raw, cond_means, cond_stds, noise_level=0.0, args=None):
+    g, means, stds, hist, nl = args or _cond_grid_args(cond_inputs, histogram_raw, cond_means, cond_stds, noise_level)
+    pos = np.ascontiguousarray(np.asarray(tiles, dtype=np.int32).reshape(-1, 2))
+    out = torch.empty((len(pos), 53 + hist.size), dtype=torch.float32, device=torch.device("cuda", engine.device_id))
+    check(lib().td_cond_rows(engine._h, ptr(g), g.shape[1], g.shape[2], len(pos), ptr(pos), ptr(means), ptr(stds), ptr(hist), hist.size, nl, ptr(out)))
+    return out
+
+
+def tile_conditioning_rows(engine, cond_inputs, tiles, histogram_raw, cond_means, cond_stds, noise_level):
+    args = _cond_grid_args(cond_inputs, histogram_raw, cond_means, cond_stds, noise_level) if engine is not None and engine.get_option("grid_fused", 1) != 0 else None
+    if args is None:
+        return _tile_conditioning(torch.as_tensor(cond_inputs, dtype=torch.float32), tiles, histogram_raw, cond_means, cond_stds, noise_level)
+    return cond_rows(engine, cond_inputs, tiles, histogram_raw, cond_means, cond_stds, noise_level, args=args)
+
+
 def blend_windows(engine, canvas, tiles, tile_idx, h_starts, w_starts, size, accumulate=True):
     C_, Hc, Wc = canvas.shape[0] - 1, canvas.shape[1], canvas.shape[2]
     rs = np.asarray(h_starts, dtype=np.int32)
@@ -181,18 +211,46 @@
     run = all_tiles if tiles is None else [t for t in all_tiles if t in set(tiles)]
     canvas = torch.zeros((C_ + 1, H, W), dtype=torch.float32, device=dev)
     windows = {}
+    grid_args = _cond_grid_args(cond_inputs, histogram_raw, cond_means, cond_stds, noise_level) if cond_inputs.ndim == 4 else None
+    fused = eng.get_option("grid_fused", 1) != 0 and (guide_model is None or guidance_scale == 1.0) and (cond_inputs.ndim == 1 or grid_args is not None)
+    nth, ntw = max(64, th), max(64, tw)
+    if fused:
+        sig = np.ascontiguousarray(scheduler.sigmas.to(torch.float32).cpu().numpy())
+        eng.set_option("solver_order", int(getattr(scheduler.config, "solver_order", 2)))
+        eng.set_option("lower_order_final", int(bool(getattr(scheduler.config, "lower_order_final", True))))
+        rs, cs = np.asarray(h_starts, dtype=np.int32), np.asarray(w_starts, dtype=np.int32)
     for b0 in range(0, len(run), max_batch):
         chunk = run[b0:b0 + max_batch]
         origins = [(noise_origin[0] + h_starts[ic], noise_origin[1] + w_starts[jc]) for ic, jc in chunk]
-        nth, ntw = max(64, th), max(64, tw)
-        x = _noise.gaussian_noise_patches(noise_seed, origins, th, tw, channels=C_, tile_h=nth, tile_w=ntw, scale=sigma0, device=dev)
-        cond = _tile_conditioning(cond_inputs, chunk, histogram_raw, cond_means, cond_stds, noise_level).to(dev).contiguous()
-        sample_tiles_edm(model, scheduler, x, cond, steps, guide_model=guide_model, guidance_scale=guidance_scale)
+        if fused:
+            org = np.ascontiguousarray(np.asarray(origins, dtype=np.int64).reshape(-1, 2))
+            _noise.check_origins(org, th, tw)
+            pos = np.ascontiguousarray(np.asarray(chunk, dtype=np.int32).reshape(-1, 2))
+            wi, wj = np.ascontiguousarray(pos[:, 0]), np.ascontiguousarray(pos[:, 1])
+            x = torch.empty((len(chunk), C_, th, tw), dtype=torch.float32, device=dev) if (return_windows or tile_size is None) else None
+            b = GridBatch(noise_seed=int(noise_seed) & _noise.M64, n=len(chunk), H=th, W=tw, tile_h=nth, tile_w=ntw, noise_scale=sigma0, origins_host=ptr(org),
+                          n_steps=steps, sigma_data=sd, sigmas_host=ptr(sig), windows_out=ptr(x))
+            if grid_args is not None:
+                g, means, stds, hist, nl = grid_args
+                b.cond_grid, b.grid_rows, b.grid_cols, b.cond_pos_host = ptr(g), g.shape[1], g.shape[2], ptr(pos)
+                b.cond_means_host, b.cond_stds_host, b.hist_host, b.n_hist, b.noise_level = ptr(means), ptr(stds), ptr(hist), hist.size, nl
+            else:
+                rows = cond_inputs.view(1, -1).expand(len(chunk), -1).contiguous()
+                b.cond_rows = ptr(rows)
+            if tile_size is not None:
+                b.canvas, b.Hc, b.Wc, b.size, b.accumulate = ptr(canvas), H, W, tile_size, 1
+                b.n_rows, b.row_starts_host, b.n_cols, b.col_starts_host, b.wi_host, b.wj_host = len(rs), ptr(rs), len(cs), ptr(cs), ptr(wi), ptr(wj)
+            check(lib().td_sample_grid_batch(model._h, C.byref(b)))
+        else:
+            x = _noise.gaussian_noise_patches(noise_seed, origins, th, tw, channels=C_, tile_h=nth, tile_w=ntw, scale=sigma0, device=dev)
+            cond = _tile_conditioning(cond_inputs, chunk, histogram_raw, cond_means, cond_stds, noise_level).to(dev).contiguous()
+            sample_tiles_edm(model, scheduler, x, cond, steps, guide_model=guide_model, guidance_scale=guidance_scale)
         if tile_size is None:
             return x
         if return_windows:
             windows.update({t: x[k].clone() for k, t in enumerate(chunk)})
-        blend_windows(eng, canvas, x, chunk, h_starts, w_starts, tile_size, accumulate=True)
+        if not fused:
+            blend_windows(eng, canvas, x, chunk, h_starts, w_starts, tile_size, accumulate=True)
     out = canvas if return_canvas else blend_normalize(eng, canvas, 1.0 / sd)[None]
     return (out, windows) if return_windows else out
 
```
